# Angtian/VoGE

Measured on AMD Instinct MI355X. Metric: forward+backward frames/sec at 512^2, 50k Gaussians; ray-trace HBM GB/s vs peak, higher is better.
Workload: dtype f32; 1 GPU; cfg3_50k_512: 50000 random Gaussians (scalar sigmas), 512x512, K=40, max_point_per_bin=-1, fwd+bwd (grads to verts, sigmas, colors); launch=hip graph replay, 4 consecutive steps per graph launch, parallelism=1 gpu

## Files before the change

voge_amd/csrc/sweep_iso.h:

```cpp
#pragma once
#include <type_traits>

#include "voge_common.h"

namespace voge {

constexpr int kS2TP = 65;
constexpr int kS2TQ = 66;
constexpr int kS2Pad = 4;

struct Sweep2Stage {
  float x[64 + kS2Pad], y[64 + kS2Pad], z[64 + kS2Pad], a[64 + kS2Pad];
  union {
    float lb[64];
    int cnt[64];
  };
  int pos[64 + kS2Pad];
};
__host__ __device__ inline size_t sweep2_len_bytes(const int K) { return (sizeof(float) * (size_t)(K + 1) * kS2TP + 15) & ~(size_t)15; }
__host__ __device__ inline size_t sweep2_pos_bytes(const int K) { return (sizeof(uint16_t) * (size_t)(K + 1) * kS2TQ + 15) & ~(size_t)15; }
struct Sweep2Gen {
  float e[11][64 + kS2Pad];
};
constexpr int kS2DiagRows = 5;
__host__ __device__ inline size_t sweep2_lds_bytes(const int K, const int gen = 0) {
  return sweep2_len_bytes(K) + sweep2_pos_bytes(K) + sizeof(Sweep2Stage) +
         (gen == 1 ? sizeof(Sweep2Gen) : (gen == 2 ? sizeof(float) * kS2DiagRows * (64 + kS2Pad) : 0));
}

#ifndef VOGE_S2_EPI_B
#define VOGE_S2_EPI_B 5
#endif
#ifndef VOGE_S2_EPI_R
#define VOGE_S2_EPI_R 3
#endif
#ifndef VOGE_S2_EXIT_GROUP
#define VOGE_S2_EXIT_GROUP 16
#endif
constexpr int kExitGroup = VOGE_S2_EXIT_GROUP;

template <int GEN>
__global__ void __launch_bounds__(64)
sweep_iso_kernel(const float4 *__restrict__ cull, const float4 *__restrict__ ms, const float4 *__restrict__ evr, const float *__restrict__ rays,
                 const int *__restrict__ bin_count, const int32_t *__restrict__ bin_id, const float *__restrict__ bin_lb,
                 const int32_t *__restrict__ tl_id, const float *__restrict__ tl_lb, const int32_t *__restrict__ pool_id,
                 const float *__restrict__ pool_lb, const int *__restrict__ tl_off, const int2 *__restrict__ order,
                 const int tiles_per_img, const int nstx, const int nst, const int N, const int H, const int W, const int K,
                 const float thr_act, int32_t *__restrict__ out_idx, float *__restrict__ out_len, float *__restrict__ out_act,
                 float *__restrict__ out_dsd, int32_t *__restrict__ out_cnt,
                 const CamView cam ) {
  extern __shared__ __attribute__((aligned(16))) unsigned char smem_raw[];
  float *const Llen = reinterpret_cast<float *>(smem_raw);
  unsigned char *const Lpos_raw = smem_raw + sweep2_len_bytes(K);
  Sweep2Stage &S = *reinterpret_cast<Sweep2Stage *>(smem_raw + sweep2_len_bytes(K) + sweep2_pos_bytes(K));
  Sweep2Gen &G = *reinterpret_cast<Sweep2Gen *>(smem_raw + sweep2_len_bytes(K) + sweep2_pos_bytes(K) + sizeof(Sweep2Stage));
  auto grow = [&](const int r) -> float * { return &G.e[GEN == 2 ? (r < 2 ? r : r - 3) : r][0]; };
  auto ghas = [](const int r) { return GEN != 2 || r < 2 || (r >= 5 && r < 8); };

  const int lane = threadIdx.x;
  const int tiles_x = (W + 7) >> 3;
#ifdef VOGE_SWEEP_TIMES
  const unsigned long long ts0 = wall_clock64();
  unsigned long long ts_fill = 0, ts_cons = 0, ts1 = 0, ts2 = 0;
  unsigned st_eval = 0;
  unsigned long long ts_slow = 0; unsigned st_slow = 0, st_lanes = 0, st_moved = 0, st_far = 0;
  int dbg_moved = 0;
#endif
  const int2 slot = order[blockIdx.x];
  if (slot.x < 0) return;
  if (slot.y == 0) {
    if (out_act != nullptr) return;
    const int lin0 = slot.x & ~kPoolFlag;
    const int b = lin0 / tiles_per_img, bx = lin0 - b * tiles_per_img;
    const int ftx = bx % tiles_x, fty = bx / tiles_x;
    const int tw = min(8, W - ftx * 8), th = min(8, H - fty * 8);
    const int row_items = tw * K;
    if ((K & 3) == 0) {
      const int ipr = row_items >> 2;
      for (int it = lane; it < th * ipr; it += 64) {
        const int rr = it / ipr, j4 = it - rr * ipr;
        const size_t o = (((size_t)b * H + fty * 8 + rr) * W + (size_t)ftx * 8) * K + (size_t)j4 * 4;
        st16i<true>(out_idx + o, -1, -1, -1, -1);
        st16f<true>(out_len + o, VOGE_SENT_LEN, VOGE_SENT_LEN, VOGE_SENT_LEN, VOGE_SENT_LEN);
      }
    } else {
      for (int it = lane; it < th * row_items; it += 64) {
        const int rr = it / row_items, j = it - rr * row_items;
        const size_t o = (((size_t)b * H + fty * 8 + rr) * W + (size_t)ftx * 8) * K + j;
        out_idx[o] = -1; out_len[o] = VOGE_SENT_LEN;
      }
    }
    if (out_cnt != nullptr) {
      const int rr = lane >> 3, x = lane & 7;
      if (rr < th && x < tw) out_cnt[((size_t)b * H + fty * 8 + rr) * W + (size_t)ftx * 8 + x] = 0;
    }
    if (cam.R != nullptr && cam.rays_out != nullptr) {
      const int rr = lane >> 3, x = lane & 7;
      if (rr < th && x < tw) {
        const CamK ck = cam_load(cam, b);
        float ex, ey, ez;
        cam_ray(ck, cam_irow(cam, fty * 8 + rr), ftx * 8 + x, ex, ey, ez);
        float *o = cam.rays_out + (((size_t)b * H + fty * 8 + rr) * W + (size_t)ftx * 8 + x) * 3;
        o[0] = ex; o[1] = ey; o[2] = ez;
      }
    }
    return;
  }
  const bool pooled = (slot.x & kPoolFlag) != 0;
  const int lin = slot.x & ~kPoolFlag;
  const int b = lin / tiles_per_img, bx = lin - b * tiles_per_img;
  const int tx = bx % tiles_x, ty = bx / tiles_x;
  const int bin = (b * nst + ((ty * 8) / kST) * nstx + (tx * 8) / kST) * 4 + (((ty * 8) / kQuad) & 1) * 2 + (((tx * 8) / kQuad) & 1);
  const int tc = slot.y;
  const int bc = (tc >= 0) ? tc : ((bin_count != nullptr) ? bin_count[bin] : -1);
  const bool binned = bc >= 0;
  const int src_n = binned ? bc : N;
  const size_t list_at = pooled ? (size_t)tl_off[lin] : (size_t)lin * kTileCap;
  const int32_t *src_id = (tc >= 0) ? (pooled ? pool_id : tl_id) + list_at : (binned ? bin_id + (size_t)bin * kQCap : nullptr);
  const float *src_lb = (tc >= 0) ? (pooled ? pool_lb : tl_lb) + list_at : (binned ? bin_lb + (size_t)bin * kQCap : nullptr);
  const bool pref = tc >= 0;
  const float4 *cullb = cull + (size_t)b * N;
  const float4 *msb = ms + (size_t)b * N;
  const float4 rec_none = make_float4(0.f, 0.f, 0.f, INFINITY);
  const float4 cull_none = make_float4(0.f, 0.f, 0.f, -1.f);
  const bool h_is_id = (N <= 65536) || !binned;
  auto id_of = [&](const unsigned h) -> int { return h_is_id ? (int)h : src_id[h]; };
  const float not_full = __uint_as_float(__float_as_uint(VOGE_SENT_LEN) - 1u);
  if (lane < kS2Pad) { S.x[64 + lane] = 0.f; S.y[64 + lane] = 0.f; S.z[64 + lane] = 0.f; S.a[64 + lane] = INFINITY; }
  if (GEN && lane < kS2Pad) G.e[0][64 + lane] = __uint_as_float(0x7fc00000u);
  const float4 *evrb = GEN ? evr + (size_t)b * N * 3 : nullptr;
  bool tile_gen = false;

  Cone wcone;
  bool unit_rays = false;
  wcone.ok = false;
  const bool from_cam = cam.R != nullptr;
  CamK ck;
  if (from_cam) ck = cam_load(cam, b);
  auto ray_of = [&](const int x, const int y, float &rx, float &ry, float &rz) {
    if (from_cam) {
      cam_ray(ck, cam_irow(cam, y), x, rx, ry, rz);
    } else {
      const size_t rid = ((size_t)b * H + y) * W + x;
      rx = rays[3 * rid + 0]; ry = rays[3 * rid + 1]; rz = rays[3 * rid + 2];
    }
  };
  auto ray_setup = [&](const bool mine, const float mdx, const float mdy, const float mdz) {
    const int px = tx * 8 + (lane & 7), py = ty * 8 + (lane >> 3);
    float ox_ = mdx, oy_ = mdy, oz_ = mdz;
    if (!mine) ray_of(min(px, W - 1), min(py, H - 1), ox_, oy_, oz_);
    const RayDir u = ray_dir(ox_, oy_, oz_);
    unit_rays = __all(!u.ok || u.unit);
    wcone.ok = false;
    if (!pref) {
      const bool dirs_ok = __all(u.ok);
      const float wsx = wave_sum_dpp(u.ok ? u.ux : 0.f), wsy = wave_sum_dpp(u.ok ? u.uy : 0.f), wsz = wave_sum_dpp(u.ok ? u.uz : 0.f);
      const float n = sqrtf(fmaf(wsz, wsz, fmaf(wsy, wsy, wsx * wsx)));
      const float ax = wsx / n, ay = wsy / n, az = wsz / n;
      float smax = 0.f, cmin = 1.f;
      cone_partial(u, ax, ay, az, smax, cmin);
      wcone = cone_finish(ax, ay, az, n, wave_max(smax), wave_min(cmin), dirs_ok);
    }
  };

  auto run = [&](auto wide_tag, const int pass) {
    constexpr bool WIDE = decltype(wide_tag)::value;
    const int r = WIDE ? pass * 32 + (lane & 31) : lane;
    const int col = WIDE ? (lane & 31) : lane;
    const int px = tx * 8 + (r & 7), py = ty * 8 + (r >> 3);
    const bool valid = (px < W) && (py < H) && (!WIDE || lane < 32);
    const size_t ray_id = ((size_t)b * H + min(py, H - 1)) * W + min(px, W - 1);
    int id0 = (lane < src_n) ? (binned ? src_id[lane] : lane) : -1;
    float lb0 = (binned && lane < src_n) ? src_lb[lane] : -INFINITY;
    int id1 = (64 + lane < src_n) ? (binned ? src_id[64 + lane] : 64 + lane) : -1;
    float lb1 = (binned && 64 + lane < src_n) ? src_lb[64 + lane] : -INFINITY;
    float dx, dy, dz;
    ray_of(min(px, W - 1), min(py, H - 1), dx, dy, dz);
    if (from_cam && cam.rays_out != nullptr && valid) {
      float *o = cam.rays_out + 3 * ray_id;
      o[0] = dx; o[1] = dy; o[2] = dz;
    }
    const __amdgpu_buffer_rsrc_t rs_ms = out_rsrc(const_cast<float4 *>(msb), (unsigned)N * 16u),
                                 rs_cull = out_rsrc(const_cast<float4 *>(cullb), (unsigned)N * 16u);
    auto load_ms = [&](const int id) {
      const voge_v4f r = __builtin_amdgcn_raw_buffer_load_b128(rs_ms, id * 16, 0, 0);
      return make_float4(r[0], r[1], r[2], (id >= 0) ? r[3] : INFINITY);
    };
    auto load_cull = [&](const int id) {
      const voge_v4f r = __builtin_amdgcn_raw_buffer_load_b128(rs_cull, id * 16, 0, 0);
      return make_float4(r[0], r[1], r[2], (id >= 0) ? r[3] : -1.f);
    };
    const __amdgpu_buffer_rsrc_t rs_ev = out_rsrc(const_cast<float4 *>(GEN ? evrb : msb), GEN ? (unsigned)N * 48u : 0u);
    auto load_ev = [&](const int id, const int k) {
      const voge_v4f r = __builtin_amdgcn_raw_buffer_load_b128(rs_ev, id * 48 + 16 * k, 0, 0);
      return make_float4(r[0], r[1], r[2], r[3]);
    };
    float4 m0 = load_ms(id0);
    float4 c0 = pref ? cull_none : load_cull(id0);
    float4 ea0 = rec_none, ea1 = rec_none, ea2 = rec_none;
    if (GEN) { ea0 = load_ev(id0, 0); ea1 = load_ev(id0, 1); ea2 = load_ev(id0, 2); }
    if (pass == 0) ray_setup(!WIDE, dx, dy, dz);
    const float rdn2 = __builtin_amdgcn_rcpf((dx * dx + dy * dy) + dz * dz);
    float *const mylen = Llen + col;
    uint16_t *const mypos16 = reinterpret_cast<uint16_t *>(Lpos_raw) + col;
    uint32_t *const mypos32 = reinterpret_cast<uint32_t *>(Lpos_raw) + col;
    auto put = [&](const int row, const float len, const unsigned p) {
      mylen[__umul24((unsigned)row, (unsigned)kS2TP)] = len;
      if (WIDE) mypos32[__umul24((unsigned)row, (unsigned)(kS2TQ / 2))] = p; else mypos16[__umul24((unsigned)row, (unsigned)kS2TQ)] = (uint16_t)p;
    };
    auto len_at = [&](const int row) -> float { return mylen[__umul24((unsigned)row, (unsigned)kS2TP)]; };
    auto pos_at = [&](const int row) -> unsigned {
      return WIDE ? mypos32[__umul24((unsigned)row, (unsigned)(kS2TQ / 2))] : (unsigned)mypos16[__umul24((unsigned)row, (unsigned)kS2TQ)];
    };

    int cnt = 0;
    float worstf = valid ? not_full : __uint_as_float(0x7fc00000u);
    float tailf = -INFINITY;
    bool wdone = false;

    auto slow_insert = [&](const float len, const unsigned p) {
      const bool full = (cnt == K);
      int my_id = -1;
      auto key_le = [&](const float pl, const int row) {
        if (pl != len) return pl < len;
        if (my_id < 0) my_id = id_of(p);
        return id_of(pos_at(row)) <= my_id;
      };
      if (full && len == worstf && key_le(worstf, K - 1)) return;
      int pos = full ? K - 1 : cnt;
      float new_tail = len;
      bool first = true;
      while (pos > 0) {
        const float pl = len_at(pos - 1);
        if (key_le(pl, pos - 1)) break;
        if (first) new_tail = pl;
        put(pos, pl, pos_at(pos - 1));
        first = false;
        --pos;
      }
      put(pos, len, p);
#ifdef VOGE_SWEEP_SLOW
      dbg_moved = (full ? K - 1 : cnt) - pos;
#endif
      if (full) {
        tailf = new_tail;
        worstf = new_tail;
      } else {
        if (pos == cnt) tailf = len;
        if (++cnt == K) worstf = tailf;
      }
    };
    auto lean_insert = [&](const float len, const unsigned p, const bool slow, const int Kv) -> bool {
      const bool full = (cnt == K);
      const int top = full ? Kv - 1 : cnt;
      const int r1 = max(top - 1, 0), r2 = max(top - 2, 0), r3 = max(top - 3, 0);
      float l1 = len_at(r1), l2 = len_at(r2), l3 = len_at(r3);
      const unsigned h1 = pos_at(r1), h2 = pos_at(r2);
      l1 = (top >= 1) ? l1 : -INFINITY; l2 = (top >= 2) ? l2 : -INFINITY; l3 = (top >= 3) ? l3 : -INFINITY;
      const bool g1 = l1 > len, g2 = g1 & (l2 > len);
      const float below = g2 ? l3 : (g1 ? l2 : l1);
      const bool ok = slow & (below < len) & !(full & (len == worstf));
      const int n = (g1 ? 1 : 0) + (g2 ? 1 : 0);
      put((ok & g1) ? top : Kv, l1, h1);
      put((ok & g2) ? top - 1 : Kv, l2, h2);
      put(ok ? top - n : Kv, len, p);
      tailf = ok ? (g1 ? l1 : len) : tailf;
      cnt += (ok & !full) ? 1 : 0;
      worstf = (ok & (cnt == K)) ? tailf : worstf;
      return slow & !ok;
    };
    int Kv = K;
    asm volatile("" : "+v"(Kv));
    auto deep_insert = [&](const float len, const unsigned p, const bool slow) {
      const bool full = (cnt == K);
      bool go = slow;
      int my_id = -1;
      if (__builtin_expect(__ballot(go & full & (len == worstf)) != 0ull, 0)) {
        if (go & full & (len == worstf)) {
          my_id = id_of(p);
          if (!(my_id < id_of(pos_at(K - 1)))) go = false;
        }
      }
      int pos = full ? K - 1 : cnt;
      const int pos0 = pos;
      float top = len;
      bool walking = go, first = true;
      while (__ballot(walking) != 0ull) {
        const int r1 = max(pos - 1, 0), r2 = max(pos - 2, 0), r3 = max(pos - 3, 0), r4 = max(pos - 4, 0);
        const float l1 = len_at(r1), l2 = len_at(r2), l3 = len_at(r3), l4 = len_at(r4);
        const unsigned h1 = pos_at(r1), h2 = pos_at(r2), h3 = pos_at(r3), h4 = pos_at(r4);
        bool g1 = l1 > len, g2 = l2 > len, g3 = l3 > len, g4 = l4 > len;
        if (__builtin_expect(__ballot(walking & ((l1 == len) | (l2 == len) | (l3 == len) | (l4 == len))) != 0ull, 0)) {
          if (walking & ((l1 == len) | (l2 == len) | (l3 == len) | (l4 == len))) {
            if (my_id < 0) my_id = id_of(p);
            g1 = g1 | ((l1 == len) && id_of(h1) > my_id); g2 = g2 | ((l2 == len) && id_of(h2) > my_id);
            g3 = g3 | ((l3 == len) && id_of(h3) > my_id); g4 = g4 | ((l4 == len) && id_of(h4) > my_id);
          }
        }
        const bool c1 = walking & (pos >= 1) & g1, c2 = c1 & (pos >= 2) & g2, c3 = c2 & (pos >= 3) & g3, c4 = c3 & (pos >= 4) & g4;
        if (first) top = c1 ? l1 : len;
        first = false;
        put(c1 ? pos : Kv, l1, h1);
        put(c2 ? pos - 1 : Kv, l2, h2);
        put(c3 ? pos - 2 : Kv, l3, h3);
        put(c4 ? pos - 3 : Kv, l4, h4);
        pos -= (c1 ? 1 : 0) + (c2 ? 1 : 0) + (c3 ? 1 : 0) + (c4 ? 1 : 0);
        walking = c4;
      }
      put(go ? pos : Kv, len, p);
      if (go) {
        if (full) {
          tailf = top; worstf = top;
        } else {
          if (pos == pos0) tailf = len;
          if (++cnt == K) worstf = tailf;
        }
      }
    };

    auto commit = [&](const float len, const float act, const unsigned p) {
      const bool take = (act < thr_act) & (len <= worstf);
      const bool app = take & (len > tailf);
      put(WIDE ? (app ? cnt : Kv) : cnt, len, p);
      cnt += app ? 1 : 0;
      tailf = app ? len : tailf;
      worstf = (app & (cnt == K)) ? len : worstf;
      const bool slow = take & !app;
      if (__builtin_expect(__ballot(slow) != 0ull, 0)) {
#ifdef VOGE_SWEEP_SLOW
        const unsigned long long tss = wall_clock64();
#endif
#ifdef VOGE_SWEEP_SLOW
        dbg_moved = 0;
#endif
        if (GEN == 1) {
          deep_insert(len, p, slow);
        } else {
          const bool hard = lean_insert(len, p, slow, Kv);
          if (__builtin_expect(__ballot(hard) != 0ull, 0)) {
            if (hard) slow_insert(len, p);
          }
        }
#ifdef VOGE_SWEEP_SLOW
        ts_slow += wall_clock64() - tss; ++st_slow;
        {
          const int nl = __popcll(__ballot(slow));
          int mx = slow ? dbg_moved : 0;
          for (int o = 32; o > 0; o >>= 1) mx = max(mx, __shfl_xor(mx, o, 64));
          st_lanes += nl; st_moved += mx; st_far += (mx >= 4) ? 1 : 0;
        }
#endif
      }
    };

    auto load_id = [&](const int g) { return (g < src_n) ? (binned ? src_id[g] : g) : -1; };
    auto load_lb = [&](const int g) { return (binned && g < src_n) ? src_lb[g] : -INFINITY; };

#ifdef VOGE_SWEEP_TIMES
    ts1 = wall_clock64();
#endif
    for (int base = 0; base < src_n && !wdone; base += 64) {
      const int id = id0;
      const float lbv = lb0;
      const float4 mrec = m0, crec = c0;
      const float4 e0 = ea0, e1 = ea1, e2 = ea2;
      id0 = id1; lb0 = lb1;
      m0 = load_ms(id0);
      c0 = pref ? cull_none : load_cull(id0);
      if (GEN) { ea0 = load_ev(id0, 0); ea1 = load_ev(id0, 1); ea2 = load_ev(id0, 2); }
      id1 = load_id(base + 128 + lane);
      lb1 = load_lb(base + 128 + lane);
#ifdef VOGE_SWEEP_TIMES
      const unsigned long long tsa = wall_clock64();
#endif
      int nbuf;
      __syncthreads();
      const bool cgen = GEN && !(mrec.w == mrec.w);
      auto stage_gen = [&](const int sl) {
        const float ev[11] = {cgen ? e0.y : __uint_as_float(0x7fc00000u), e0.z, e0.w, e1.x, e1.y, e1.z, e1.w, e2.x, e2.y, e2.z, e2.w};
#pragma unroll
        for (int r = 0; r < 11; ++r)
          if (ghas(r)) grow(r)[sl] = ev[r];
      };
      const float a_st = cgen ? e0.x : mrec.w;
      if (pref) {
        S.x[lane] = mrec.x; S.y[lane] = mrec.y; S.z[lane] = mrec.z; S.a[lane] = a_st;
        S.lb[lane] = lbv;
        S.pos[lane] = h_is_id ? id : base + lane;
        if (GEN) stage_gen(lane);
        nbuf = min(64, src_n - base);
      } else {
        const bool keep = cone_keep(crec, wcone);
        const unsigned long long m = __ballot(keep);
        nbuf = __popcll(m);
        if (keep) {
          const int sl = __popcll(m & ((1ull << lane) - 1ull));
          S.x[sl] = mrec.x; S.y[sl] = mrec.y; S.z[sl] = mrec.z; S.a[sl] = a_st;
          S.lb[sl] = lbv;
          S.pos[sl] = h_is_id ? id : base + lane;
          if (GEN) stage_gen(sl);
        }
        if (lane < kS2Pad) { S.x[nbuf + lane] = 0.f; S.y[nbuf + lane] = 0.f; S.z[nbuf + lane] = 0.f; S.a[nbuf + lane] = INFINITY; }
        if (GEN && lane < kS2Pad) G.e[0][nbuf + lane] = __uint_as_float(0x7fc00000u);
      }
      __syncthreads();
      unsigned long long gmask = 0ull;
      unsigned long long dmask = 0ull;
      if (GEN) {
        const float mk = G.e[0][lane];
        gmask = __ballot(lane < nbuf && mk == mk);
        tile_gen = tile_gen || gmask != 0ull;
        if (GEN == 2) {
          dmask = gmask;
        } else if (gmask != 0ull) {
          const bool dg = G.e[2][lane] == 0.0f && G.e[3][lane] == 0.0f && G.e[4][lane] == 0.0f && G.e[8][lane] == 0.0f &&
                          G.e[9][lane] == 0.0f && G.e[10][lane] == 0.0f;
          dmask = __ballot(lane < nbuf && mk == mk && dg);
        }
      }
      const bool chunk_diag = GEN && gmask != 0ull && dmask == gmask;
#ifdef VOGE_SWEEP_TIMES
      const unsigned long long tsb = wall_clock64();
      ts_fill += tsb - tsa;
#endif
      const float lbl = S.lb[lane];
      int n = nbuf;
      float4 Xn = *reinterpret_cast<const float4 *>(&S.x[0]), Yn = *reinterpret_cast<const float4 *>(&S.y[0]),
             Zn = *reinterpret_cast<const float4 *>(&S.z[0]), An = *reinterpret_cast<const float4 *>(&S.a[0]);
      int4 Pn = *reinterpret_cast<const int4 *>(&S.pos[0]);
      float4 Evn[GEN ? 11 : 1];
      if (GEN) {
#pragma unroll
        for (int r = 0; r < 11; ++r) Evn[GEN ? r : 0] = ghas(r) ? *reinterpret_cast<const float4 *>(grow(r)) : make_float4(0.f, 0.f, 0.f, 0.f);
        if (GEN != 2 && chunk_diag) {
#pragma unroll
          for (int r = 0; r < 11; ++r)
            if (!(r < 2 || (r >= 5 && r < 8))) Evn[GEN ? r : 0] = make_float4(0.f, 0.f, 0.f, 0.f);
        }
      }
      for (int s0 = 0; s0 < n; s0 += 4) {
        if ((s0 & (kExitGroup - 1)) == 0 && binned && unit_rays && __all(!valid || cnt == K)) {
          const float wmax = wave_max(valid ? worstf : -INFINITY);
          const unsigned long long ex = __ballot(lane < nbuf && lbl > wmax);
          if (ex) {
            n = __builtin_ctzll(ex);
            wdone = true;
            if (n <= s0) break;
          }
        }
        const float4 X = Xn, Y = Yn, Z = Zn, A = An;
        const int4 P = Pn;
        const int pv[4] = {P.x, P.y, P.z, P.w};
        float len[4], act[4];
        const unsigned gbits = GEN ? (unsigned)(gmask >> s0) & 15u : 0u;
        if (GEN && gbits != 0u) {
          float4 Ev[11];
#pragma unroll
          for (int r = 0; r < 11; ++r) Ev[r] = Evn[GEN ? r : 0];
          const float qxx = dx * dx, qyy = dy * dy, qzz = dz * dz, qxy = dx * dy, qxz = dx * dz, qyz = dy * dz;
          if (gbits == 15u && ((unsigned)(dmask >> s0) & 15u) == 15u) {
#pragma unroll
            for (int h = 0; h < 2; ++h) {
              auto half = [&](const float4 v) { return h ? (v2f){v.z, v.w} : (v2f){v.x, v.y}; };
              const v2f x2 = half(X), y2 = half(Y), z2 = half(Z), s00 = half(A), s11 = half(Ev[0]), s22 = half(Ev[1]),
                        bx = half(Ev[5]), by = half(Ev[6]), bz = half(Ev[7]);
              v2f ksk = s00 * splat(qxx);
              ksk = pk_fma(s11, splat(qyy), ksk); ksk = pk_fma(s22, splat(qzz), ksk);
              v2f msk = bx * splat(dx);
              msk = pk_fma(by, splat(dy), msk); msk = pk_fma(bz, splat(dz), msk);
              const v2f t = msk * (v2f){__builtin_amdgcn_rcpf(ksk.x), __builtin_amdgcn_rcpf(ksk.y)} + splat(0.0f);
              const v2f vx = pk_fma(-t, splat(dx), x2), vy = pk_fma(-t, splat(dy), y2), vz = pk_fma(-t, splat(dz), z2);
              v2f a = s00 * (vx * vx);
              a = pk_fma(s11, vy * vy, a); a = pk_fma(s22, vz * vz, a);
              len[2 * h] = t.x; len[2 * h + 1] = t.y;
              act[2 * h] = a.x; act[2 * h + 1] = a.y;
            }
          } else if (GEN != 2 && gbits == 15u) {
#pragma unroll
            for (int h = 0; h < 2; ++h) {
              auto half = [&](const float4 v) { return h ? (v2f){v.z, v.w} : (v2f){v.x, v.y}; };
              const v2f x2 = half(X), y2 = half(Y), z2 = half(Z), s00 = half(A), s11 = half(Ev[0]), s22 = half(Ev[1]), s01 = half(Ev[2]),
                        s02 = half(Ev[3]), s12 = half(Ev[4]), bx = half(Ev[5]), by = half(Ev[6]), bz = half(Ev[7]), kx = half(Ev[8]),
                        ky = half(Ev[9]), kz = half(Ev[10]);
              v2f ksk = s00 * splat(qxx);
              ksk = pk_fma(s11, splat(qyy), ksk); ksk = pk_fma(s22, splat(qzz), ksk); ksk = pk_fma(s01, splat(qxy), ksk);
              ksk = pk_fma(s02, splat(qxz), ksk); ksk = pk_fma(s12, splat(qyz), ksk);
              v2f msk = bx * splat(dx);
              msk = pk_fma(by, splat(dy), msk); msk = pk_fma(bz, splat(dz), msk);
              const v2f t = msk * (v2f){__builtin_amdgcn_rcpf(ksk.x), __builtin_amdgcn_rcpf(ksk.y)} + splat(0.0f);
              const v2f vx = pk_fma(-t, splat(dx), x2), vy = pk_fma(-t, splat(dy), y2), vz = pk_fma(-t, splat(dz), z2);
              v2f a = s00 * (vx * vx);
              a = pk_fma(s11, vy * vy, a); a = pk_fma(s22, vz * vz, a); a = pk_fma(s01, vx * vy, a);
              a = pk_fma(s02, vx * vz, a); a = pk_fma(s12, vy * vz, a);
              v2f kd = kx * splat(dx);
              kd = pk_fma(ky, splat(dy), kd); kd = pk_fma(kz, splat(dz), kd);
              a = pk_fma(t, kd, a);
              len[2 * h] = t.x; len[2 * h + 1] = t.y;
              act[2 * h] = a.x; act[2 * h + 1] = a.y;
            }
          } else {
            const float mxs[4] = {X.x, X.y, X.z, X.w}, mys[4] = {Y.x, Y.y, Y.z, Y.w}, mzs[4] = {Z.x, Z.y, Z.z, Z.w}, avs[4] = {A.x, A.y, A.z, A.w};
#pragma unroll
            for (int q = 0; q < 4; ++q) {
              auto el = [&](const float4 v) { return q == 0 ? v.x : (q == 1 ? v.y : (q == 2 ? v.z : v.w)); };
              if ((gbits >> q) & 1u) {
                EvalRec e;
                e.s00 = avs[q]; e.s11 = el(Ev[0]); e.s22 = el(Ev[1]); e.s01 = el(Ev[2]); e.s02 = el(Ev[3]); e.s12 = el(Ev[4]);
                e.bx = el(Ev[5]); e.by = el(Ev[6]); e.bz = el(Ev[7]); e.kx = el(Ev[8]); e.ky = el(Ev[9]); e.kz = el(Ev[10]);
                const PairOut o = pair_eval_gen(mxs[q], mys[q], mzs[q], e, dx, dy, dz, qxx, qyy, qzz, qxy, qxz, qyz);
                len[q] = o.len; act[q] = o.act;
              } else {
                const float md = fmaf(mzs[q], dz, fmaf(mys[q], dy, mxs[q] * dx));
                const float t = md * rdn2;
                const float vx = fmaf(-t, dx, mxs[q]), vy = fmaf(-t, dy, mys[q]), vz = fmaf(-t, dz, mzs[q]);
                len[q] = t;
                act[q] = avs[q] * fmaf(vz, vz, fmaf(vy, vy, vx * vx));
              }
            }
          }
        } else {
#pragma unroll
        for (int h = 0; h < 2; ++h) {
          const v2f x2 = h ? (v2f){X.z, X.w} : (v2f){X.x, X.y}, y2 = h ? (v2f){Y.z, Y.w} : (v2f){Y.x, Y.y},
                    z2 = h ? (v2f){Z.z, Z.w} : (v2f){Z.x, Z.y}, a2 = h ? (v2f){A.z, A.w} : (v2f){A.x, A.y};
          const v2f md = pk_fma(z2, splat(dz), pk_fma(y2, splat(dy), x2 * splat(dx)));
          const v2f t = md * splat(rdn2);
          const v2f vx = pk_fma(-t, splat(dx), x2), vy = pk_fma(-t, splat(dy), y2), vz = pk_fma(-t, splat(dz), z2);
          const v2f a = a2 * pk_fma(vz, vz, pk_fma(vy, vy, vx * vx));
          len[2 * h] = t.x; len[2 * h + 1] = t.y;
          act[2 * h] = a.x; act[2 * h + 1] = a.y;
        }
        }
#pragma unroll
        for (int q = 0; q < 4; ++q) asm volatile("" : "+v"(len[q]), "+v"(act[q]));
        Xn = *reinterpret_cast<const float4 *>(&S.x[s0 + 4]); Yn = *reinterpret_cast<const float4 *>(&S.y[s0 + 4]);
        Zn = *reinterpret_cast<const float4 *>(&S.z[s0 + 4]); An = *reinterpret_cast<const float4 *>(&S.a[s0 + 4]);
        Pn = *reinterpret_cast<const int4 *>(&S.pos[s0 + 4]);
        if (GEN && chunk_diag) {
#pragma unroll
          for (int r = 0; r < 11; ++r)
            if (r < 2 || (r >= 5 && r < 8)) Evn[GEN ? r : 0] = *reinterpret_cast<const float4 *>(grow(r) + s0 + 4);
        } else if (GEN == 1 && gmask != 0ull) {
#pragma unroll
          for (int r = 0; r < 11; ++r) Evn[GEN ? r : 0] = *reinterpret_cast<const float4 *>(&G.e[r][s0 + 4]);
        }
#pragma unroll
        for (int q = 0; q < 4; ++q) commit(len[q], act[q], (unsigned)pv[q]);
      }
#ifdef VOGE_SWEEP_TIMES
      ts_cons += wall_clock64() - tsb;
      st_eval += min(n, nbuf);
#endif
    }
#ifdef VOGE_SWEEP_TIMES
    ts2 = wall_clock64();
#endif

    __syncthreads();
    S.cnt[lane] = valid ? cnt : 0;
    if (out_cnt != nullptr && valid) out_cnt[((size_t)b * H + py) * W + px] = cnt;
    __syncthreads();
    const int row0 = WIDE ? pass * 4 : 0;
    const int th = max(0, min(WIDE ? 4 : 8, H - ty * 8 - row0)), tw = min(8, W - tx * 8);
    const int row_items = tw * K;
    const uint16_t *const P16 = reinterpret_cast<const uint16_t *>(Lpos_raw);
    const uint32_t *const P32 = reinterpret_cast<const uint32_t *>(Lpos_raw);
    auto entry_pos = [&](const int s, const int owner) -> unsigned {
      return WIDE ? P32[s * (kS2TQ / 2) + owner] : (unsigned)P16[s * kS2TQ + owner];
    };
    const bool want_ad = out_act != nullptr;
    const int gofs = b * N;
    if ((K & 3) == 0) {
      constexpr int kEpiB = VOGE_S2_EPI_B, kEpiR = VOGE_S2_EPI_R;
      const int ipr = row_items >> 2, nitem = th * ipr;
      const float inv_ipr = 1.0f / (float)max(ipr, 1), invK = 1.0f / (float)K;
      const size_t tile_pix = ((size_t)b * H + ty * 8 + row0) * W + (size_t)tx * 8;
      int32_t *const t_idx = out_idx + tile_pix * K;
      float *const t_len = out_len + tile_pix * K;
      const unsigned h_last = (unsigned)max(src_n - 1, 0);
      const bool wt_ok = (size_t)W * (size_t)K < ((size_t)1 << 26);
      const unsigned rs_bytes = wt_ok ? (unsigned)th * (unsigned)W * (unsigned)K * 4u : 0u;
      const __amdgpu_buffer_rsrc_t rs_idx = out_rsrc(t_idx, rs_bytes), rs_len = out_rsrc(t_len, rs_bytes);
      for (int it0 = lane; it0 < nitem; it0 += 64 * kEpiB) {
        int32_t oi[kEpiB][4];
        float ol[kEpiB][4];
        unsigned rel[kEpiB];
        int nv[kEpiB];
#pragma unroll
        for (int u = 0; u < kEpiB; ++u) {
          const int it = it0 + u * 64;
          const bool in = it < nitem;
          const int itc = in ? it : 0;
          const int rr = __float2int_rz(((float)itc + 0.5f) * inv_ipr);
          const int j = (itc - rr * ipr) * 4;
          const int x = __float2int_rz(((float)j + 0.5f) * invK);
          const int sl = j - x * K;
          const int owner = rr * 8 + x;
          rel[u] = (unsigned)(rr * W + x) * (unsigned)K + (unsigned)sl;
          nv[u] = in ? max(0, min(4, S.cnt[owner] - sl)) : -1;
#pragma unroll
          for (int q = 0; q < 4; ++q) {
            const float l = Llen[(sl + q) * kS2TP + owner];
            const unsigned h = entry_pos(sl + q, owner);
            ol[u][q] = (q < nv[u]) ? l : VOGE_SENT_LEN;
            oi[u][q] = (int)h;
          }
        }
        if (h_is_id) {
#pragma unroll
          for (int u = 0; u < kEpiB; ++u)
#pragma unroll
            for (int q = 0; q < 4; ++q) oi[u][q] = (q < nv[u]) ? oi[u][q] + gofs : -1;
        } else {
          int idv[kEpiB][4];
#pragma unroll
          for (int u = 0; u < kEpiB; ++u)
#pragma unroll
            for (int q = 0; q < 4; ++q) idv[u][q] = src_id[min((unsigned)oi[u][q], h_last)];
#pragma unroll
          for (int u = 0; u < kEpiB; ++u)
#pragma unroll
            for (int q = 0; q < 4; ++q) oi[u][q] = (q < nv[u]) ? idv[u][q] + gofs : -1;
        }
        if (!want_ad) {
#pragma unroll
          for (int u = 0; u < kEpiB; ++u) {
            if (nv[u] < 0) continue;
            if (wt_ok) {
              st16i_wt(rs_idx, rel[u] * 4u, oi[u][0], oi[u][1], oi[u][2], oi[u][3]);
              st16f_wt(rs_len, rel[u] * 4u, ol[u][0], ol[u][1], ol[u][2], ol[u][3]);
            } else {
              st16i<false>(t_idx + rel[u], oi[u][0], oi[u][1], oi[u][2], oi[u][3]);
              st16f<false>(t_len + rel[u], ol[u][0], ol[u][1], ol[u][2], ol[u][3]);
            }
          }
        } else if (GEN && tile_gen) {
          float *const t_act = out_act + tile_pix * K, *const t_dsd = out_dsd + tile_pix * K;
#pragma unroll
          for (int u = 0; u < kEpiB; ++u) {
            const unsigned pr = rel[u] / (unsigned)K;
            const float *ry = rays + (tile_pix + pr) * 3;
            const float ex = ry[0], ey = ry[1], ez = ry[2];
            float4 rc[4], g0[4], g1[4], g2[4];
#pragma unroll
            for (int q = 0; q < 4; ++q) {
              const size_t gi = (size_t)((q < nv[u]) ? oi[u][q] : gofs);
              rc[q] = ms[gi]; g0[q] = evr[gi * 3]; g1[q] = evr[gi * 3 + 1]; g2[q] = evr[gi * 3 + 2];
            }
            float oa[4], od[4];
            const float dn2 = (ex * ex + ey * ey) + ez * ez;
#pragma unroll
            for (int q = 0; q < 4; ++q) {
              PairOut o;
              if (rc[q].w == rc[q].w) o = pair_eval_iso_at(rc[q].x, rc[q].y, rc[q].z, rc[q].w, ol[u][q], ex, ey, ez, dn2);
              else o = pair_eval_gen(rc[q].x, rc[q].y, rc[q].z, unpack_eval(g0[q], g1[q], g2[q]), ex, ey, ez, ex * ex, ey * ey, ez * ez,
                                     ex * ey, ex * ez, ey * ez);
              oa[q] = (q < nv[u]) ? o.act : VOGE_SENT_ACT;
              od[q] = (q < nv[u]) ? o.dsd : 0.0f;
            }
            if (nv[u] < 0) continue;
            st16i<true>(t_idx + rel[u], oi[u][0], oi[u][1], oi[u][2], oi[u][3]);
            st16f<true>(t_len + rel[u], ol[u][0], ol[u][1], ol[u][2], ol[u][3]);
            st16f<true>(t_act + rel[u], oa[0], oa[1], oa[2], oa[3]);
            st16f<true>(t_dsd + rel[u], od[0], od[1], od[2], od[3]);
          }
        } else {
          float *const t_act = out_act + tile_pix * K, *const t_dsd = out_dsd + tile_pix * K;
#pragma unroll
          for (int u0 = 0; u0 < kEpiB; u0 += kEpiR) {
            float4 rec[kEpiR][4];
            float ex[kEpiR], ey[kEpiR], ez[kEpiR];
#pragma unroll
            for (int v = 0; v < kEpiR; ++v) {
              const int u = u0 + v;
              if (u >= kEpiB) continue;
              const unsigned pr = rel[u] / (unsigned)K;
              const float *ry = rays + (tile_pix + pr) * 3;
              ex[v] = ry[0]; ey[v] = ry[1]; ez[v] = ry[2];
#pragma unroll
              for (int q = 0; q < 4; ++q) rec[v][q] = ms[(q < nv[u]) ? oi[u][q] : gofs];
            }
#pragma unroll
            for (int v = 0; v < kEpiR; ++v) {
              const int u = u0 + v;
              if (u >= kEpiB) continue;
              float oa[4], od[4];
              const float dn2 = (ex[v] * ex[v] + ey[v] * ey[v]) + ez[v] * ez[v];
#pragma unroll
              for (int q = 0; q < 4; ++q) {
                const PairOut o = pair_eval_iso_at(rec[v][q].x, rec[v][q].y, rec[v][q].z, rec[v][q].w, ol[u][q], ex[v], ey[v], ez[v], dn2);
                oa[q] = (q < nv[u]) ? o.act : VOGE_SENT_ACT;
                od[q] = (q < nv[u]) ? o.dsd : 0.0f;
              }
              if (nv[u] < 0) continue;
              st16i<true>(t_idx + rel[u], oi[u][0], oi[u][1], oi[u][2], oi[u][3]);
              st16f<true>(t_len + rel[u], ol[u][0], ol[u][1], ol[u][2], ol[u][3]);
              st16f<true>(t_act + rel[u], oa[0], oa[1], oa[2], oa[3]);
              st16f<true>(t_dsd + rel[u], od[0], od[1], od[2], od[3]);
            }
          }
        }
      }
    } else {
      constexpr int kOddU = 8;
      const float inv_ri = 1.0f / (float)max(row_items, 1), invK = 1.0f / (float)K;
      const int nit = th * row_items;
      const size_t tile_pix = ((size_t)b * H + ty * 8 + row0) * W + (size_t)tx * 8;
      int32_t *const t_idx = out_idx + tile_pix * K;
      float *const t_len = out_len + tile_pix * K;
      const unsigned h_last = (unsigned)max(src_n - 1, 0);
      for (int it0 = lane; it0 < nit; it0 += kOddU * 64) {
        int32_t oi[kOddU];
        float ol[kOddU];
        unsigned rel[kOddU], pr[kOddU];
        bool in[kOddU], on[kOddU];
#pragma unroll
        for (int u = 0; u < kOddU; ++u) {
          const int it = it0 + u * 64;
          on[u] = it < nit;
          const int itc = on[u] ? it : 0;
          const int rr = __float2int_rz(((float)itc + 0.5f) * inv_ri);
          const int j = itc - rr * row_items;
          const int x = __float2int_rz(((float)j + 0.5f) * invK);
          const int sl = j - x * K;
          const int owner = rr * 8 + x;
          pr[u] = (unsigned)(rr * W + x);
          rel[u] = pr[u] * (unsigned)K + (unsigned)sl;
          in[u] = on[u] && sl < S.cnt[owner];
          ol[u] = Llen[sl * kS2TP + owner];
          oi[u] = (int)entry_pos(sl, owner);
        }
        if (h_is_id) {
#pragma unroll
          for (int u = 0; u < kOddU; ++u) oi[u] = in[u] ? oi[u] + gofs : -1;
        } else {
          int idv[kOddU];
#pragma unroll
          for (int u = 0; u < kOddU; ++u) idv[u] = src_id[min((unsigned)oi[u], h_last)];
#pragma unroll
          for (int u = 0; u < kOddU; ++u) oi[u] = in[u] ? idv[u] + gofs : -1;
        }
#pragma unroll
        for (int u = 0; u < kOddU; ++u) ol[u] = in[u] ? ol[u] : VOGE_SENT_LEN;
        if (!want_ad) {
#pragma unroll
          for (int u = 0; u < kOddU; ++u)
            if (on[u]) { t_idx[rel[u]] = oi[u]; t_len[rel[u]] = ol[u]; }
        } else {
          float *const t_act = out_act + tile_pix * K, *const t_dsd = out_dsd + tile_pix * K;
          float oa[kOddU], od[kOddU];
#pragma unroll
          for (int u = 0; u < kOddU; ++u) {
            const float *ry = rays + (tile_pix + pr[u]) * 3;
            const float ex = ry[0], ey = ry[1], ez = ry[2];
            const size_t gi = (size_t)(in[u] ? oi[u] : gofs);
            const float4 cc = ms[gi];
            PairOut o;
            if (GEN && tile_gen && !(cc.w == cc.w)) {
              o = pair_eval_gen(cc.x, cc.y, cc.z, unpack_eval(evr[gi * 3], evr[gi * 3 + 1], evr[gi * 3 + 2]), ex, ey, ez, ex * ex, ey * ey,
                                ez * ez, ex * ey, ex * ez, ey * ez);
            } else {
              o = pair_eval_iso_at(cc.x, cc.y, cc.z, cc.w, ol[u], ex, ey, ez, (ex * ex + ey * ey) + ez * ez);
            }
            oa[u] = in[u] ? o.act : VOGE_SENT_ACT; od[u] = in[u] ? o.dsd : 0.0f;
          }
#pragma unroll
          for (int u = 0; u < kOddU; ++u)
            if (on[u]) { t_idx[rel[u]] = oi[u]; t_len[rel[u]] = ol[u]; t_act[rel[u]] = oa[u]; t_dsd[rel[u]] = od[u]; }
        }
      }
    }
  };

  if ((h_is_id ? N : src_n) <= 65536) {
    run(std::false_type{}, 0);
  } else {
    run(std::true_type{}, 0);
    run(std::true_type{}, 1);
  }
#ifdef VOGE_SWEEP_TIMES
  if (lane == 0 && b == 0 && bx < 8192) {
    unsigned long long *o = g_sweep_times + 8 * (size_t)bx;
    o[0] = ts0; o[1] = ts1; o[2] = ts_fill; o[3] = ts_cons; o[4] = ts2; o[5] = wall_clock64(); o[6] = ((unsigned long long)blockIdx.x << 32) | st_eval;
#ifdef VOGE_SWEEP_SLOW
    o[7] = (ts_slow << 32) | st_slow;
    o[2] = ((unsigned long long)st_far << 48) | ((unsigned long long)(st_moved & 0xffffu) << 32) | st_lanes;
#else
    o[7] = (unsigned long long)__builtin_amdgcn_s_getreg((4 << 0) | (0 << 6) | (31 << 11)) |
           ((unsigned long long)__builtin_amdgcn_s_getreg((20 << 0) | (0 << 6) | (31 << 11)) << 32);
#endif
  }
#endif
}

}
```

voge_amd/csrc/trace_bin.h:

```cpp
#pragma once
#include <type_traits>

#include "voge_common.h"

namespace voge {

constexpr int kST0 = 128;
constexpr int kCh = kST0 / kST;
constexpr int kBinThreads = 1024;
constexpr int kParts = 16;
constexpr int kSegCap = 512;
constexpr int kTileCap = 2048;
constexpr int kTilesPerBin = (kST / 8) * (kST / 8);
constexpr int kRankMaxBins = 4096;
static_assert(kCh * kCh == kBinThreads / 64, "one wave per super-tile of a region / per sweep tile of a super-tile");

__device__ __forceinline__ float depth_key(const float4 c, const Cone &k) {
  const float nm = __builtin_amdgcn_sqrtf(fmaf(c.z, c.z, fmaf(c.y, c.y, c.x * c.x)));
  const float R = c.w;
  if (!(R < 3e38f) || !(nm < 3e38f)) return -INFINITY;
  float kappa = -nm;
  if (k.ok && k.cs >= 0.5f && nm > 4.0f * R) {
    const float p = fmaf(c.z, k.az, fmaf(c.y, k.ay, c.x * k.ax));
    if (p > 0.0f) kappa = nm;
  }
  return kappa;
}

__device__ __forceinline__ float4 iso_cull_record(const float mx, const float my, const float mz, const float a,
                                                  const float thr_act) {
  float reach = INFINITY;
  if (a > 0.0f && a < 3e38f) {
    const float nm = __builtin_amdgcn_sqrtf(fmaf(mz, mz, fmaf(my, my, mx * mx)));
    const float r = __builtin_amdgcn_sqrtf(fmaxf(thr_act, 0.0f) * __builtin_amdgcn_rcpf(a * (1.0f - 4e-6f))) * (1.0f + 2e-5f) + 2e-5f * nm + 1e-30f;
    reach = r;
    if (!(reach >= 0.0f)) reach = INFINITY;
    if (reach < 3e38f) reach = __uint_as_float((__float_as_uint(reach) + 1u) & ~1u);
  }
  return make_float4(mx, my, mz, reach);
}

#ifdef VOGE_BIN_TIMES
__device__ unsigned long long g_bin_times[2][1024 * 8];
__device__ unsigned long long g_bin_wave[1024 * 16 * 4];
#define BIN_WTS(k) \
  if ((threadIdx.x & 63) == 0 && blockIdx.y == 0 && blockIdx.x < 1024) g_bin_wave[(blockIdx.x * 16 + (threadIdx.x >> 6)) * 4 + (k)] = wall_clock64()
#define BIN_TS(which, k) \
  if (threadIdx.x == 0 && blockIdx.y == 0 && blockIdx.x < 1024) g_bin_times[which][8 * blockIdx.x + (k)] = wall_clock64()
#else
#define BIN_TS(which, k)
#define BIN_WTS(k)
#endif

constexpr int kRoundChunks = 4;
constexpr int kRoundCap = kRoundChunks * kBinThreads;

constexpr int kExtMul = 3;
constexpr int kExtChunk = 1024;
constexpr int kExtChunks = 16;
__host__ __device__ inline int slice_cap(const int N) {
  return ((N + kParts * kBinThreads - 1) / (kParts * kBinThreads)) * kBinThreads;
}
struct BinALds {
  int arena_top;
  int extc[kCh * kCh][kExtChunks];
  int extn[kCh * kCh];
  float4 srec[kRoundCap];
  int sid[kRoundCap];
  ConeRec child[kCh * kCh];
  ConeRec region;
  ConeRec rowc[kCh];
  int use_rows;
  int cnt0[kRoundChunks][16];
  int base[kCh * kCh];
  int nS;
};

struct BinARaw {
  float4 v;
};
struct BinAView {
  float ox, oy, oz;
  float fx, fy, fz;
  bool has_f;
};
template <bool ISO_PREP>
__device__ __forceinline__ BinAView binA_view(const int b, const float *__restrict__ cam_fwd, const IsoView view,
                                              const CamView &cam = no_camera(), const CamK *ck = nullptr) {
  BinAView V;
  V.ox = V.oy = V.oz = 0.f; V.fx = V.fy = V.fz = 0.f; V.has_f = false;
  if (ISO_PREP) {
    if (view.origin != nullptr) { const float *o = view.origin + 3 * b; V.ox = o[0]; V.oy = o[1]; V.oz = o[2]; }
    if (cam_fwd != nullptr) { const float *f = cam_fwd + 3 * b; V.fx = f[0]; V.fy = f[1]; V.fz = f[2]; V.has_f = true; }
    if (cam.R != nullptr) {
      cam_origin(*ck, cam.T + 3 * b, V.ox, V.oy, V.oz);
      if (cam.behind) { const float *r = cam.R + 9 * b; V.fx = r[2]; V.fy = r[5]; V.fz = r[8]; V.has_f = true; }
    }
  }
  return V;
}
template <bool ISO_PREP>
__device__ __forceinline__ BinARaw binA_fetch(const int g, const int b, const int N, const float4 *__restrict__ cull,
                                              const float *__restrict__ mus, const float *__restrict__ isg, const IsoView view) {
  BinARaw r;
  r.v = make_float4(0.f, 0.f, 0.f, 0.f);
  if (N <= 0) return r;
  const int gc = max(g, 0);
  if (!ISO_PREP) { r.v = cull[(size_t)b * N + gc]; return r; }
  const size_t src = view.shared ? (size_t)gc : (size_t)b * N + gc;
  r.v = make_float4(mus[3 * src + 0], mus[3 * src + 1], mus[3 * src + 2], isg[src]);
  return r;
}
template <bool ISO_PREP>
__device__ __forceinline__ float4 binA_derive(const BinARaw r, const bool valid, const BinAView &V, const float thr_act,
                                              const IsoView view, float &a_out) {
  a_out = 0.f;
  if (!valid) return make_float4(0.f, 0.f, 0.f, -1.f);
  if (!ISO_PREP) return r.v;
  float mx = r.v.x, my = r.v.y, mz = r.v.z;
  if (view.origin != nullptr || view.cam_origin) { mx -= V.ox; my -= V.oy; mz -= V.oz; }
  const float a = iso_view_a(r.v.w, view.mode);
  a_out = a;
  float4 c = iso_cull_record(mx, my, mz, a, thr_act);
  if (V.has_f && fmaf(mz, V.fz, fmaf(my, V.fy, mx * V.fx)) < 0.0f) c.w = -1.0f;
  return c;
}

__host__ __device__ inline bool deal_interleaved(const int N) { return N < kParts * kBinThreads; }
__device__ __forceinline__ int slice_of(const int g, const int N) {
  return deal_interleaved(N) ? g % kParts : (g / kBinThreads) % kParts;
}

template <bool ISO_PREP>
__global__ void __launch_bounds__(kBinThreads)
binA_kernel(const ConeRec *__restrict__ cones , const int nstx, const int nsty, const int nst0x,
            const float *__restrict__ mus, const float *__restrict__ isg, const float *__restrict__ cam_fwd, const int N,
            const float thr_act, const IsoView view, float4 *__restrict__ cull, float4 *__restrict__ ms,
            int *__restrict__ seg_count , int32_t *__restrict__ seg_id ,
            float4 *__restrict__ seg_rec ,
            unsigned long long *__restrict__ pool_top ,
            int *__restrict__ seg_ext ,
            int32_t *__restrict__ ext_id , const int ext_arena,
            const CamView cam ) {
  __shared__ BinALds L;
  const int tid = threadIdx.x, lane = tid & 63, wave = tid >> 6;
  const int region = blockIdx.x / kParts, part = blockIdx.x - region * kParts;
  const int b = blockIdx.y;
  if (blockIdx.x == 0 && blockIdx.y == 0 && tid == 0) *pool_top = 0ull;
  const int rx = region % nst0x, ry = region / nst0x;
  const int nst = nstx * nsty;
  if (tid < kCh * kCh) { L.base[tid] = 0; L.extn[tid] = 0; }
  if (tid == 0) L.arena_top = 0;
  int32_t *const arena = ext_id + ((size_t)(b * (int)(gridDim.x / kParts) + region) * kParts + part) * (size_t)ext_arena;
  int ext_have = 0;
  BIN_TS(0, 0);
  const bool interleaved = deal_interleaved(N);
  const int nchunks = interleaved ? kParts * ((N + kParts * kBinThreads - 1) / (kParts * kBinThreads))
                                  : (N + kBinThreads - 1) / kBinThreads;
  const bool writes_records = ISO_PREP && region == 0;
  float4 c[kRoundChunks];
  float av[kRoundChunks];
  int gq[kRoundChunks];
  CamK ck;
  if (cam.R != nullptr) ck = cam_load(cam, b);
  const BinAView V = binA_view<ISO_PREP>(b, cam_fwd, view, cam, &ck);
  if (cam.R != nullptr && cam.origin_out != nullptr && blockIdx.x == 0 && tid == 0) {
    float ox = V.ox, oy = V.oy, oz = V.oz;
    if (!ISO_PREP) cam_origin(ck, cam.T + 3 * b, ox, oy, oz);
    cam.origin_out[3 * b] = ox; cam.origin_out[3 * b + 1] = oy; cam.origin_out[3 * b + 2] = oz;
  }
  BinARaw raw[kRoundChunks];
  auto fetch_round = [&](const int j0) {
#pragma unroll
    for (int q = 0; q < kRoundChunks; ++q) {
      const int j = j0 + q * kParts;
      const int g = interleaved ? ((j / kParts) * kBinThreads + tid) * kParts + part : j * kBinThreads + tid;
      gq[q] = (j < nchunks && g < N) ? g : -1;
      raw[q] = binA_fetch<ISO_PREP>(gq[q], b, N, cull, mus, isg, view);
    }
  };
  auto derive_round = [&]() {
#pragma unroll
    for (int q = 0; q < kRoundChunks; ++q) c[q] = binA_derive<ISO_PREP>(raw[q], gq[q] >= 0, V, thr_act, view, av[q]);
  };
  auto load_round = [&](const int j0) { fetch_round(j0); derive_round(); };
  fetch_round(part);
  if (wave == 0) {
    const int cc = lane & (kCh * kCh - 1);
    const int cx = rx * kCh + (cc & (kCh - 1)), cy = ry * kCh + cc / kCh;
    ConeRec r = {0.f, 0.f, 1.f, 1.f, 0.f, -1.f, 0.f, 0.f};
    const bool region_rect = cam.R != nullptr && cam.h <= cam.stripe_h;
    if (cam.R != nullptr) {
      const bool reg = region_rect && lane == kCh * kCh;
      const int j0 = reg ? rx * kCh * kST : cx * kST, i0 = reg ? ry * kCh * kST : cy * kST, ext = reg ? kCh * kST : kST;
      if ((cx < nstx && cy < nsty) || reg) r = cam_rect_cone(ck, cam, j0, j0 + ext - 1, i0, i0 + ext - 1);
    } else if (cx < nstx && cy < nsty) {
      r = cones[cone_super_at(b, nst, cy * nstx + cx)];
    }
    if (lane < kCh * kCh) L.child[lane] = r;
    if (region_rect) {
      if (lane == kCh * kCh) L.region = r;
      if (lane == 0) L.use_rows = 0;
    } else {
    const bool present = lane < kCh * kCh && r.ok >= 0.f;
    const float sx = wave_sum_dpp(present ? r.ax : 0.f), sy = wave_sum_dpp(present ? r.ay : 0.f), sz = wave_sum_dpp(present ? r.az : 0.f);
    const float npres = wave_sum_dpp(present ? 1.f : 0.f);
    bool ok = __all(!present || r.ok > 0.f);
    const float n = sqrtf(fmaf(sz, sz, fmaf(sy, sy, sx * sx)));
    const float ax = sx / n, ay = sy / n, az = sz / n;
    auto child_extrema = [&](const float ax_, const float ay_, const float az_, float &smax_, float &cmin_, bool &ok_) {
      smax_ = 0.f; cmin_ = 1.f;
      if (present) {
        const float ca = fmaf(r.az, az_, fmaf(r.ay, ay_, r.ax * ax_));
        const float qx = fmaf(-ca, ax_, r.ax), qy = fmaf(-ca, ay_, r.ay), qz = fmaf(-ca, az_, r.az);
        const float sa = sqrtf(fmaf(qz, qz, fmaf(qy, qy, qx * qx))) * (1.0f + 1e-6f) + 1e-7f;
        const float cl = fminf(ca, 1.0f) - 1e-7f;
        if (!(cl > 0.0f)) ok_ = false;
        cmin_ = fmaf(cl, r.cs, -sa * r.sn);
        smax_ = fmaf(fminf(ca + 1e-7f, 1.0f), r.sn, sa);
      }
    };
    float smax, cmin;
    child_extrema(ax, ay, az, smax, cmin, ok);
    ok = __all(ok);
    smax = wave_max(smax); cmin = wave_min(cmin);
    const Cone cn = cone_finish(ax, ay, az, n / fmaxf(npres, 1.f), smax, cmin, ok);
    if (lane == 0) L.region = ConeRec{cn.ax, cn.ay, cn.az, cn.cs, cn.sn, cn.ok ? 1.f : 0.f, 0.f, 0.f};
    const float widest_child = wave_max(present ? (r.ok > 0.f ? r.sn : 2.0f) : 0.f);
    if (lane == 0) L.use_rows = 0;
    if (__builtin_expect((!cn.ok || cn.sn > 8.0f * widest_child) && N < (1 << 27), 0)) {
      auto quad_sum = [](float v) { v += VOGE_DPP(v, 0xB1); v += VOGE_DPP(v, 0x4E); return v; };
      auto quad_max = [](float v) { v = fmaxf(v, VOGE_DPP(v, 0xB1)); v = fmaxf(v, VOGE_DPP(v, 0x4E)); return v; };
      auto quad_min = [](float v) { v = fminf(v, VOGE_DPP(v, 0xB1)); v = fminf(v, VOGE_DPP(v, 0x4E)); return v; };
      static_assert(kCh == 4, "a row of super-tiles is a DPP quad");
      const float qsx = quad_sum(present ? r.ax : 0.f), qsy = quad_sum(present ? r.ay : 0.f), qsz = quad_sum(present ? r.az : 0.f);
      const float qn = quad_sum(present ? 1.f : 0.f);
      const float nn = sqrtf(fmaf(qsz, qsz, fmaf(qsy, qsy, qsx * qsx)));
      const float rax = qsx / nn, ray = qsy / nn, raz = qsz / nn;
      float rs, rc;
      bool rok = !present || r.ok > 0.f;
      child_extrema(rax, ray, raz, rs, rc, rok);
      rs = quad_max(rs); rc = quad_min(rc);
      const float okf = quad_min(rok ? 1.f : 0.f);
      const Cone rcn = cone_finish(rax, ray, raz, nn / fmaxf(qn, 1.f), rs, rc, okf != 0.f);
      if (lane < kCh * kCh && (lane & 3) == 0) L.rowc[lane >> 2] = ConeRec{rcn.ax, rcn.ay, rcn.az, rcn.cs, rcn.sn, qn > 0.f ? (rcn.ok ? 1.f : 0.f) : -1.f, 0.f, 0.f};
      const float widest_row = wave_max((lane < kCh * kCh && qn > 0.f) ? (rcn.ok ? rcn.sn : 2.0f) : 0.f);
      if (lane == 0) L.use_rows = (!cn.ok || cn.sn > 1.6f * widest_row) ? 1 : 0;
    }
    }
  }
  BIN_TS(0, 6);
  derive_round();
  BIN_TS(0, 7);
  __syncthreads();
  const Cone rcone = load_cone(L.region);
  const bool use_rows = L.use_rows != 0;
  BIN_TS(0, 1);

  auto rounds = [&](auto rows_tag) {
    constexpr bool ROWS = decltype(rows_tag)::value;
    for (int j0 = part; j0 < nchunks; j0 += kParts * kRoundChunks) {
      if (j0 != part) load_round(j0);
      bool k0[kRoundChunks];
      unsigned rowm[kRoundChunks];
  #pragma unroll
      for (int q = 0; q < kRoundChunks; ++q) {
        if (writes_records && gq[q] >= 0) {
          cull[(size_t)b * N + gq[q]] = c[q];
          ms[(size_t)b * N + gq[q]] = make_float4(c[q].x, c[q].y, c[q].z, av[q]);
        }
        k0[q] = cone_keep(c[q], rcone);
        rowm[q] = 0xFu;
        if (ROWS) {
          rowm[q] = 0u;
  #pragma unroll
          for (int g = 0; g < kCh; ++g) {
            const ConeRec rr = L.rowc[g];
            if (rr.ok >= 0.f && cone_keep(c[q], load_cone(rr))) rowm[q] |= 1u << g;
          }
          k0[q] = rowm[q] != 0u;
        }
      }
      unsigned long long m0[kRoundChunks];
  #pragma unroll
      for (int q = 0; q < kRoundChunks; ++q) {
        m0[q] = __ballot(k0[q]);
        if (lane == 0) L.cnt0[q][wave] = __popcll(m0[q]);
      }
      __syncthreads();
      static_assert(kRoundChunks * 16 == 64, "one lane per (chunk, wave)");
      int nS;
      int my_off[kRoundChunks];
      {
        const int v = (&L.cnt0[0][0])[lane];
        const int x = wave_incl_scan_i32(v);
        nS = __builtin_amdgcn_readlane(x, 63);
  #pragma unroll
        for (int q = 0; q < kRoundChunks; ++q) my_off[q] = __shfl(x - v, q * 16 + wave, 64);
      }
  #pragma unroll
      for (int q = 0; q < kRoundChunks; ++q)
        if (k0[q]) {
          const int pos = my_off[q] + __popcll(m0[q] & ((1ull << lane) - 1ull));
          L.srec[pos] = c[q];
          L.sid[pos] = ROWS ? (gq[q] | (int)(rowm[q] << 27)) : gq[q];
        }
      __syncthreads();
      BIN_TS(0, 2);
      {
        const int cc = wave;
        const ConeRec cr = L.child[cc];
        if (cr.ok >= 0.f) {
          const Cone ck = load_cone(cr);
          const int ccx = rx * kCh + (cc & (kCh - 1)), ccy = ry * kCh + cc / kCh;
          const size_t seg0 = (((size_t)b * nst + ccy * nstx + ccx) * kParts + part) * kSegCap;
          int32_t *seg = seg_id + seg0;
          float4 *segr = seg_rec + seg0;
          int fill = L.base[cc];
          constexpr int kU = 4;
          for (int s0 = 0; s0 < nS; s0 += 64 * kU) {
            float4 r[kU];
            int id[kU];
  #pragma unroll
            for (int q = 0; q < kU; ++q) {
              const int si = s0 + q * 64 + lane;
              r[q] = (si < nS) ? L.srec[si] : make_float4(0.f, 0.f, 0.f, -1.f);
              id[q] = (si < nS) ? L.sid[si] : -1;
            }
            bool kp[kU];
  #pragma unroll
            for (int q = 0; q < kU; ++q) {
              bool in_row = true;
              if (ROWS) {
                in_row = id[q] >= 0 && (((unsigned)id[q] >> (27 + (cc >> 2))) & 1u) != 0u;
                id[q] = (id[q] >= 0) ? (id[q] & 0x07ffffff) : -1;
              }
              kp[q] = in_row && cone_keep(r[q], ck);
            }
            const int fill0 = fill;
  #pragma unroll
            for (int q = 0; q < kU; ++q) {
              const unsigned long long m = __ballot(kp[q]);
              if (kp[q]) {
                const int pos = fill + __popcll(m & ((1ull << lane) - 1ull));
                if (pos < kSegCap) { seg[pos] = id[q]; segr[pos] = r[q]; }
              }
              fill += __popcll(m);
            }
            if (__builtin_expect(fill > kSegCap, 0)) {
              const int need = (fill - kSegCap + kExtChunk - 1) / kExtChunk;
              while (ext_have >= 0 && ext_have < need) {
                int at = 0;
                if (lane == 0) at = atomicAdd(&L.arena_top, kExtChunk);
                at = __builtin_amdgcn_readfirstlane(at);
                if (ext_have < kExtChunks && at + kExtChunk <= ext_arena) {
                  if (lane == 0) L.extc[cc][ext_have] = at;
                  ++ext_have;
                } else {
                  ext_have = -1;
                }
              }
              wave_lds_sync();
              if (ext_have >= 0) {
                int f = fill0;
  #pragma unroll
                for (int q = 0; q < kU; ++q) {
                  const unsigned long long m = __ballot(kp[q]);
                  const int e = f + __popcll(m & ((1ull << lane) - 1ull)) - kSegCap;
                  if (kp[q] && e >= 0) arena[*lds_volatile(&L.extc[cc][e / kExtChunk]) + (e % kExtChunk)] = id[q];
                  f += __popcll(m);
                }
              }
            }
          }
          if (lane == 0) { L.base[cc] = fill; L.extn[cc] = ext_have; }
        }
      }
      BIN_TS(0, 3);
      __syncthreads();
      BIN_TS(0, 4);
    }
  };
  if (__builtin_expect(!use_rows, 1)) rounds(std::false_type{}); else rounds(std::true_type{});
  BIN_TS(0, 5);
  if (tid < kCh * kCh) {
    const int ccx = rx * kCh + (tid & (kCh - 1)), ccy = ry * kCh + tid / kCh;
    if (ccx < nstx && ccy < nsty) {
      const size_t so = ((size_t)b * nst + ccy * nstx + ccx) * kParts + part;
      const bool over = L.base[tid] > kSegCap;
      seg_count[so] = (over && L.extn[tid] < 0) ? -1 : L.base[tid];
      if (over && L.extn[tid] > 0)
        for (int q = 0; q < L.extn[tid]; ++q) seg_ext[so * kExtChunks + q] = (int)(arena - ext_id) + L.extc[tid][q];
    }
  }
}

constexpr int kQuad = 16;
constexpr int kQT = 256;
constexpr int kQCap = 3008;
constexpr int kQRec = kQCap / 2;
constexpr int kBuckets = 512;
constexpr int kTilesPerQuad = 4;
constexpr int kPoolFlag = 1 << 30;
struct BinLds {
  union {
    uint64_t keys[kQCap];
    float4 rec[kQRec];
    int hist4[kTilesPerQuad][kBuckets];
  };
  uint32_t sorted[kQCap];
  float red[4 * 8];
  union {
    int hist[kBuckets];
    int exto[kParts][kExtChunks];
  };
  uint32_t bmin[kBuckets];
  int wsum[8];
  int segn[kParts + 1];
  int extn[kParts + 1];
  unsigned ovf;
  int count;
  int nflag;
  int spill;
  float tc[kTilesPerQuad][8];
  int toff[kTilesPerQuad];
};

#ifndef VOGE_BINB_GU
#define VOGE_BINB_GU 8
#endif
constexpr int kGU = VOGE_BINB_GU;

struct BinStream {
  const float4 *cullb, *ellb, *segr;
  const int32_t *segs, *ext_id;
  const int *exto;
  int n_src, n_ext, N;
  unsigned ovf;
  Cone qcone;
};
template <bool ELL, class Sink>
__device__ __forceinline__ void bin_test_batch(const BinStream &S, const int (&gid)[kGU], const float4 (&c)[kGU], Sink &&sink) {
  bool kp[kGU], el[kGU];
  float gkey[kGU];
#pragma unroll
  for (int j = 0; j < kGU; ++j) {
    kp[j] = cone_keep(c[j], S.qcone);
    el[j] = ELL && kp[j] && cull_has_ell(c[j]);
    gkey[j] = 0.0f;
    if (ELL && __any(el[j])) {
      if (el[j]) {
        const float4 e0 = S.ellb[2 * (size_t)gid[j]], e1 = S.ellb[2 * (size_t)gid[j] + 1];
        kp[j] = cone_keep_ell(c[j], e0, e1, S.qcone);
        el[j] = kp[j];
        const float pa = fmaf(c[j].z, S.qcone.az, fmaf(c[j].y, S.qcone.ay, c[j].x * S.qcone.ax));
        gkey[j] = pa + 0.0f;
      }
    }
  }
  sink(gid, c, kp, el, gkey);
}
template <bool ELL, class Sink>
__device__ __forceinline__ void bin_stream_sources(const BinStream &S, const int *segn , const int tid, Sink &&sink) {
  int seg_p = 0, seg_lo = 0, seg_hi = segn[1];
  for (int base = 0; base < S.n_src; base += kQT * kGU) {
    int gid[kGU];
    float4 c[kGU];
#pragma unroll
    for (int j = 0; j < kGU; ++j) {
      const int i = base + j * kQT + tid;
      gid[j] = -1;
      c[j] = make_float4(0.f, 0.f, 0.f, -1.f);
      if (i < S.n_src) {
        while (i >= seg_hi) { seg_lo = seg_hi; ++seg_p; seg_hi = segn[seg_p + 1]; }
        const int o = seg_p * kSegCap + (i - seg_lo);
        gid[j] = S.segs[o];
        c[j] = S.segr[o];
      }
    }
    bin_test_batch<ELL>(S, gid, c, sink);
  }
  if (S.n_ext > 0) {
    const int *extn = segn + (kParts + 1), *exto = S.exto;
    for (int base = 0; base < S.n_ext; base += kQT * kGU) {
      int gid[kGU];
      float4 c[kGU];
#pragma unroll
      for (int j = 0; j < kGU; ++j) {
        const int i = base + j * kQT + tid;
        gid[j] = -1;
        if (i < S.n_ext) {
          int p = 0;
#pragma unroll
          for (int q = 1; q < kParts; ++q) p += (i >= extn[q]) ? 1 : 0;
          const int e = i - extn[p];
          gid[j] = S.ext_id[(size_t)exto[p * kExtChunks + e / kExtChunk] + (size_t)(e % kExtChunk)];
        }
      }
#pragma unroll
      for (int j = 0; j < kGU; ++j) c[j] = (gid[j] >= 0) ? S.cullb[gid[j]] : make_float4(0.f, 0.f, 0.f, -1.f);
      bin_test_batch<ELL>(S, gid, c, sink);
    }
  }
  if (S.ovf != 0u) {
    for (int base = 0; base < S.N; base += kQT * kGU) {
      int gid[kGU];
      float4 c[kGU];
#pragma unroll
      for (int j = 0; j < kGU; ++j) {
        const int g = base + j * kQT + tid;
        const bool ok = g < S.N && ((S.ovf >> slice_of(g, S.N)) & 1u) != 0u;
        gid[j] = ok ? g : -1;
        c[j] = ok ? S.cullb[g] : make_float4(0.f, 0.f, 0.f, -1.f);
      }
      bin_test_batch<ELL>(S, gid, c, sink);
    }
  }
}
__device__ __forceinline__ void bin_batch_slots(int *count , const int lane, const bool (&kp)[kGU], int (&slot)[kGU]) {
  unsigned long long m[kGU];
  int cw = 0;
#pragma unroll
  for (int j = 0; j < kGU; ++j) { m[j] = __ballot(kp[j]); cw += __popcll(m[j]); }
  int start = 0;
  if (cw > 0) {
    if (lane == 0) start = atomicAdd(count, cw);
    start = __builtin_amdgcn_readfirstlane(start);
  }
#pragma unroll
  for (int j = 0; j < kGU; ++j) {
    slot[j] = start + __popcll(m[j] & ((1ull << lane) - 1ull));
    start += __popcll(m[j]);
  }
}
struct BinKeys {
  float lo, scale, span, slack;
  bool flagged;
};
__device__ __forceinline__ int bin_bucket_of(const BinKeys &Kk, const float v) {
  return (v > -INFINITY) ? 1 + min(kBuckets - 2, max(0, (int)((v - Kk.lo) * Kk.scale))) : 0;
}
__device__ __forceinline__ float bin_own_bound(const BinStream &S, const size_t g) {
  const float4 cj = S.cullb[g], e0 = S.ellb[2 * g], e1 = S.ellb[2 * g + 1];
  float bnd = -INFINITY;
  if (S.qcone.ok) {
    const float pa = fmaf(cj.z, S.qcone.az, fmaf(cj.y, S.qcone.ay, cj.x * S.qcone.ax));
    const float nm1 = fabsf(cj.x) + fabsf(cj.y) + fabsf(cj.z);
    const float t = pa - ell_support(e0, e1, S.qcone.ax, S.qcone.ay, S.qcone.az) - 4e-6f * nm1;
    bnd = (t >= 0.0f) ? t : t / S.qcone.cs;
    bnd = bnd - 1e-5f * fabsf(bnd) - 1e-30f;
  }
  return bnd;
}
__device__ __forceinline__ void bin_bmin_suffix(uint32_t *bmin, int *wsum, const int tid) {
  const int lane = tid & 63, wave = tid >> 6;
  uint32_t m4[2];
#pragma unroll
  for (int q = 0; q < 2; ++q) m4[q] = bmin[2 * tid + q];
  m4[0] = min(m4[0], m4[1]);
  uint32_t x = m4[0];
#pragma unroll
  for (int o = 1; o < 64; o <<= 1) {
    const uint32_t y = __shfl_down(x, o, 64);
    if (lane + o < 64) x = min(x, y);
  }
  if (lane == 0) wsum[4 + wave] = (int)x;
  __syncthreads();
  uint32_t later = 0xffffffffu;
  {
    const uint32_t nxt = __shfl_down(x, 1, 64);
    later = (lane < 63) ? nxt : 0xffffffffu;
    for (int w = wave + 1; w < 4; ++w) later = min(later, (uint32_t)wsum[4 + w]);
  }
#pragma unroll
  for (int q = 0; q < 2; ++q) bmin[2 * tid + q] = min(m4[q], later);
}
__device__ __forceinline__ float bin_len_bound(const BinKeys &Kk, const uint32_t *bmin, const float v) {
  float edge = -INFINITY;
  int qb = 0;
  if (v > -INFINITY) {
    const int q = min(kBuckets - 2, max(0, (int)((v - Kk.lo) * Kk.scale)));
    edge = fminf(v, Kk.lo + (float)q * (Kk.span / (float)(kBuckets - 2)) - 4e-6f * Kk.span);
    qb = 1 + q;
  }
  const float lb_sphere = (edge > -INFINITY) ? edge - Kk.slack - 1e-5f * fabsf(edge) - 1e-30f : -INFINITY;
  return Kk.flagged ? fminf(lb_sphere, ord2f(bmin[qb])) : lb_sphere;
}

struct BinLong {
  BinStream S;
  BinKeys Kk;
  Cone tcone;
  bool tile_ok;
  int tile, quad, total;
  unsigned long long *pool_top;
  int *tl_off, *tl_count, *q_count;
  const int *seg_ext;
  int bin;
  int pool_cap;
  int32_t *pool_id;
  float *pool_lb;
  int2 *my_order;
};
template <bool ELL>
__device__ __forceinline__ void binB_long_path(const BinLong A, BinLds &L) {
  const int tid = threadIdx.x, lane = tid & 63, wave = tid >> 6;
  const BinStream &S = A.S;
  const int total = A.total;
  __syncthreads();
  for (int i = tid; i < kTilesPerQuad * kBuckets; i += kQT) (&L.hist4[0][0])[i] = 0;
  if (S.n_ext > 0) {
    const int p = tid / kExtChunks, q = tid % kExtChunks;
    const int ne = L.extn[p + 1] - L.extn[p];
    L.exto[p][q] = (q * kExtChunk < ne) ? A.seg_ext[((size_t)A.bin * kParts + p) * kExtChunks + q] : 0;
  }
  if (lane == 0) {
    L.tc[wave][0] = A.tcone.ax; L.tc[wave][1] = A.tcone.ay; L.tc[wave][2] = A.tcone.az; L.tc[wave][3] = A.tcone.cs;
    L.tc[wave][4] = A.tcone.sn; L.tc[wave][5] = (A.tcone.ok || !A.tile_ok) ? 1.0f : 0.0f;
    L.tc[wave][6] = A.tile_ok ? 1.0f : 0.0f;
  }
  if (tid == 0) {
    const unsigned long long at64 = atomicAdd(A.pool_top, (unsigned long long)total);
    int at = (at64 + (unsigned long long)total <= (unsigned long long)A.pool_cap) ? (int)at64 : -1;
    L.toff[0] = at;
    L.count = 0;
  }
  __syncthreads();
  const int surv_at = L.toff[0];
  bool pooled = surv_at >= 0;
  int tile_n[kTilesPerQuad] = {0, 0, 0, 0};
  if (pooled) {
    int32_t *sv_id = A.pool_id + surv_at;
    float *sv_key = A.pool_lb + surv_at;
    bin_stream_sources<ELL>(S, L.segn, tid, [&](const int (&g)[kGU], const float4 (&cj)[kGU], const bool (&kp)[kGU],
                                            const bool (&el)[kGU], const float (&gkey)[kGU]) {
      int slot[kGU];
      bin_batch_slots(&L.count, lane, kp, slot);
#pragma unroll
      for (int j = 0; j < kGU; ++j) {
        if (kp[j]) {
          sv_id[slot[j]] = (int32_t)((uint32_t)g[j] | (el[j] ? 0x80000000u : 0u));
          sv_key[slot[j]] = el[j] ? gkey[j] : depth_key(cj[j], S.qcone);
        }
      }
    });
    __threadfence_block();
    __syncthreads();
    BIN_TS(1, 2);
    auto tile_mask = [&](const size_t g, const float4 cj, const bool el) {
      unsigned mk = 0u;
#pragma unroll 1
      for (int t = 0; t < kTilesPerQuad; ++t) {
        Cone tk;
        tk.ax = L.tc[t][0]; tk.ay = L.tc[t][1]; tk.az = L.tc[t][2]; tk.cs = L.tc[t][3]; tk.sn = L.tc[t][4];
        tk.ok = L.tc[t][5] != 0.0f;
        bool k2 = (L.tc[t][6] != 0.0f) && cone_keep(cj, tk);
        if (k2 && el) k2 = cone_keep_ell(cj, S.ellb[2 * g], S.ellb[2 * g + 1], tk);
        mk |= k2 ? (1u << t) : 0u;
      }
      return mk;
    };
    for (int i = tid; i < total; i += kQT) {
      const uint32_t word = (uint32_t)sv_id[i];
      const size_t g = word & 0x7fffffffu;
      const bool el = ELL && (word & 0x80000000u) != 0u;
      const int q = bin_bucket_of(A.Kk, sv_key[i]);
      const unsigned mk = tile_mask(g, S.cullb[g], el);
#pragma unroll
      for (int t = 0; t < kTilesPerQuad; ++t)
        if ((mk >> t) & 1u) atomicAdd(&L.hist4[t][q], 1);
      if (el) atomicMin(&L.bmin[q], f2ord(bin_own_bound(S, g)));
    }
    __syncthreads();
    for (int t = 0; t < kTilesPerQuad; ++t) {
      const int2 v = *reinterpret_cast<const int2 *>(&L.hist4[t][2 * tid]);
      const int s4 = v.x + v.y;
      int x = s4;
#pragma unroll
      for (int o = 1; o < 64; o <<= 1) {
        const int y = __shfl_up(x, o, 64);
        if (lane >= o) x += y;
      }
      if (lane == 63) L.wsum[wave] = x;
      __syncthreads();
      int off = x - s4;
      for (int w = 0; w < wave; ++w) off += L.wsum[w];
      tile_n[t] = L.wsum[0] + L.wsum[1] + L.wsum[2] + L.wsum[3];
      *reinterpret_cast<int2 *>(&L.hist4[t][2 * tid]) = make_int2(off, off + v.x);
      __syncthreads();
    }
    if (ELL && A.Kk.flagged) bin_bmin_suffix(L.bmin, L.wsum, tid);
    if (tid == 0) {
      const int need = tile_n[0] + tile_n[1] + tile_n[2] + tile_n[3];
      const unsigned long long at64 = (need > 0) ? atomicAdd(A.pool_top, (unsigned long long)need) : 0ull;
      int at = (at64 + (unsigned long long)need <= (unsigned long long)A.pool_cap) ? (int)at64 : -1;
#pragma unroll
      for (int t = 0; t < kTilesPerQuad; ++t) { L.toff[t] = at; if (at >= 0) at += tile_n[t]; }
    }
    __syncthreads();
    pooled = L.toff[0] >= 0;
    BIN_TS(1, 3);
    if (pooled) {
      for (int i = tid; i < total; i += kQT) {
        const uint32_t word = (uint32_t)sv_id[i];
        const size_t g = word & 0x7fffffffu;
        const bool el = ELL && (word & 0x80000000u) != 0u;
        const float kv = sv_key[i];
        const int q = bin_bucket_of(A.Kk, kv);
        const unsigned mk = tile_mask(g, S.cullb[g], el);
        if (mk == 0u) continue;
        const float lbv = bin_len_bound(A.Kk, L.bmin, kv);
#pragma unroll
        for (int t = 0; t < kTilesPerQuad; ++t) {
          if ((mk >> t) & 1u) {
            const size_t pos = (size_t)L.toff[t] + (size_t)atomicAdd(&L.hist4[t][q], 1);
            A.pool_id[pos] = (int32_t)g;
            A.pool_lb[pos] = lbv;
          }
        }
      }
    }
  }
  if (lane == 0 && A.tile_ok) {
    A.tl_count[A.tile] = pooled ? tile_n[wave] : -1;
    A.tl_off[A.tile] = pooled ? L.toff[wave] : -1;
  }
  __syncthreads();
  if (lane == 0) L.wsum[wave] = A.tile_ok ? (pooled ? tile_n[wave] : 0x7fffffff) : -1;
  __syncthreads();
  if (lane == 0) {
    const int mine = L.wsum[wave];
    int slot = 0;
    for (int w = 0; w < kTilesPerQuad; ++w) {
      const int o = L.wsum[w];
      slot += (o > mine || (o == mine && w < wave)) ? 1 : 0;
    }
    A.my_order[slot] = make_int2(A.tile_ok ? (pooled ? (A.tile | kPoolFlag) : A.tile) : -1, pooled ? mine : -1);
  }
  if (tid == 0) A.q_count[A.quad] = pooled ? -2 : -1;
  BIN_TS(1, 4);
}


#ifndef VOGE_BINB_WPE
#define VOGE_BINB_WPE 4
#endif
template <bool ELL>
__global__ void __launch_bounds__(kQT) __attribute__((amdgpu_waves_per_eu(VOGE_BINB_WPE, VOGE_BINB_WPE)))
binB_kernel(const float4 *__restrict__ cull, const float4 *__restrict__ ell, const int *__restrict__ seg_count,
            const int32_t *__restrict__ seg_id, const float4 *__restrict__ seg_rec,
            const ConeRec *__restrict__ cones ,
            const int N, const int H, const int W,
            const int nstx, const int nsty, const int nbin_total,
            int *__restrict__ q_count, int32_t *__restrict__ q_id, float *__restrict__ q_lb,
            int *__restrict__ tl_count, int32_t *__restrict__ tl_id, float *__restrict__ tl_lb,
            int2 *__restrict__ order ,
            unsigned long long *__restrict__ pool_top, const int pool_cap, int32_t *__restrict__ pool_id, float *__restrict__ pool_lb,
            int *__restrict__ tl_off, const int *__restrict__ seg_ext, const int32_t *__restrict__ ext_id,
            const int K, int32_t *__restrict__ out_idx, float *__restrict__ out_len, float *__restrict__ out_act,
            float *__restrict__ out_dsd, int32_t *__restrict__ out_cnt, float *__restrict__ out_weight,
            int64_t *__restrict__ out_valid, const CamView cam ) {
  __shared__ BinLds L;
  const int tid = threadIdx.x, lane = tid & 63, wave = tid >> 6;
  BIN_TS(1, 7);
  const int b = blockIdx.y;
  const int binl = blockIdx.x >> 2, qq = blockIdx.x & 3;
  const int stx = binl % nstx, sty = binl / nstx;
  const int bin = b * nstx * nsty + binl;
  const int quad = bin * 4 + qq;
  const int tiles_x = (W + 7) >> 3, tiles_y = (H + 7) >> 3;
  const int tx = stx * (kST / 8) + (qq & 1) * 2 + (wave & 1), ty = sty * (kST / 8) + (qq >> 1) * 2 + (wave >> 1);
  const bool tile_ok = tx < tiles_x && ty < tiles_y;
  const int tile = b * tiles_x * tiles_y + ty * tiles_x + tx;

  ConeRec tcr, qcr;
  if (cam.R != nullptr) {
    const CamK ck = cam_load(cam, b);
    cam_two_cones(ck, cam, tx * 8, ty * 8, 8, stx * kST + (qq & 1) * kQuad, sty * kST + (qq >> 1) * kQuad, kQuad, tcr, qcr);
  } else {
    tcr = cones[cone_tile_at(b, (size_t)nstx * nsty, binl, ((qq >> 1) * 2 + (wave >> 1)) * 4 + (qq & 1) * 2 + (wave & 1))];
    qcr = cones[cone_quad_at(b, (size_t)nstx * nsty, binl, qq)];
  }
  const int my_cnt = (tid < kParts) ? seg_count[(size_t)bin * kParts + tid] : 0;
  const bool ranked = nbin_total <= kRankMaxBins;
  const int4 est0 = (ranked && tid < nbin_total) ? *reinterpret_cast<const int4 *>(seg_count + (size_t)tid * kParts) : make_int4(0, 0, 0, 0);
  const int4 est_mine = ranked ? *reinterpret_cast<const int4 *>(seg_count + (size_t)bin * kParts) : make_int4(0, 0, 0, 0);
  const Cone tcone = load_cone(tcr), qcone = load_cone(qcr);
  {
    if (tid == 0) { L.count = 0; L.nflag = 0; L.spill = 0; }
    if (wave == 0) {
      int c = (lane < kParts) ? my_cnt : 0;
      const unsigned long long ofm = __ballot(lane < kParts && c < 0);
      if (c < 0) c = 0;
      int e = 0;
      if (c > kSegCap) { e = c - kSegCap; c = kSegCap; }
      int xc = c, xe = e;
#pragma unroll
      for (int o = 1; o < kParts; o <<= 1) {
        const int yc = __shfl_up(xc, o, 64), ye = __shfl_up(xe, o, 64);
        if (lane >= o) { xc += yc; xe += ye; }
      }
      if (lane < kParts) { L.segn[lane] = xc - c; L.extn[lane] = xe - e; }
      if (lane == kParts - 1) { L.segn[kParts] = xc; L.extn[kParts] = xe; }
      if (lane == 0) L.ovf = (unsigned)ofm;
    }
    __syncthreads();
    auto load_ext_tables = [&]() {
      static_assert(kParts * kExtChunks == kQT, "one thread per (slice, chunk)");
      const int p = tid / kExtChunks, q = tid % kExtChunks;
      const int ne = L.extn[p + 1] - L.extn[p];
      L.exto[p][q] = (q * kExtChunk < ne) ? seg_ext[((size_t)bin * kParts + p) * kExtChunks + q] : 0;
    };
    if (L.extn[kParts] > 0) load_ext_tables();
  }
  BIN_TS(1, 0);

  BIN_TS(1, 6);
  int rank = bin;
  {
    auto est_of = [](const int4 v) {
      return (v.x < 0 ? kSegCap : v.x) + (v.y < 0 ? kSegCap : v.y) + (v.z < 0 ? kSegCap : v.z) + (v.w < 0 ? kSegCap : v.w);
    };
    auto estimate = [&](const int q) { return est_of(*reinterpret_cast<const int4 *>(seg_count + (size_t)q * kParts)); };
    if (ranked) {
      const int mine = est_of(est_mine);
      int ahead = 0;
      for (int q = tid; q < nbin_total; q += kQT) {
        const int e = (q == tid) ? est_of(est0) : estimate(q);
        ahead += (e > mine || (e == mine && q < bin)) ? 1 : 0;
      }
      ahead = (int)wave_sum_dpp((float)ahead);
      if (lane == 0) L.wsum[wave] = ahead;
      __syncthreads();
      rank = L.wsum[0] + L.wsum[1] + L.wsum[2] + L.wsum[3];
      __syncthreads();
    }
  }
  int2 *my_order = order + (size_t)rank * kTilesPerBin + qq * kTilesPerQuad;
  const int n_src = L.segn[kParts];
  const unsigned ovf = L.ovf;
  const float4 *cullb = cull + (size_t)b * N;
  const float4 *ellb = ell + (size_t)b * N * 2;
  const int32_t *segs = seg_id + (size_t)bin * kParts * kSegCap;
  const float4 *segr = seg_rec + (size_t)bin * kParts * kSegCap;
  float rmax = 0.0f;
  float klo = INFINITY, khi = -INFINITY;
  bool any_el = false;
  BinStream S;
  S.cullb = cullb; S.ellb = ellb; S.segr = segr; S.segs = segs; S.n_src = n_src; S.N = N; S.ovf = ovf; S.qcone = qcone;
  S.ext_id = ext_id; S.n_ext = L.extn[kParts]; S.exto = &L.exto[0][0];
  bin_stream_sources<ELL>(S, L.segn, tid, [&](const int (&g)[kGU], const float4 (&cj)[kGU], const bool (&kp)[kGU],
                                          const bool (&el)[kGU], const float (&gkey)[kGU]) {
    int slot[kGU];
    bin_batch_slots(&L.count, lane, kp, slot);
#pragma unroll
    for (int j = 0; j < kGU; ++j) {
      if (kp[j]) {
        if (!el[j] && cj[j].w < 3e38f) rmax = fmaxf(rmax, cj[j].w);
        const float kv = el[j] ? gkey[j] : depth_key(cj[j], qcone);
        if (kv > -INFINITY) { klo = fminf(klo, kv); khi = fmaxf(khi, kv); }
        if (slot[j] < kQCap) L.keys[slot[j]] = ((uint64_t)f2ord(kv) << 32) | (uint32_t)g[j] | (el[j] ? 0x80000000u : 0u);
        any_el = any_el || el[j];
      }
    }
  });
  BIN_TS(1, 1);
  if (__any(any_el) && lane == 0) L.nflag = 1;
  float hi = wave_max(khi), lo = wave_min(klo), rm = wave_max(rmax);
  if (lane == 0) { L.red[wave * 8 + 0] = hi; L.red[wave * 8 + 1] = lo; L.red[wave * 8 + 2] = rm; }
  if (S.n_ext > 0) __syncthreads();
  for (int i = tid; i < kBuckets; i += kQT) { L.hist[i] = 0; L.bmin[i] = f2ord(INFINITY); }
  __syncthreads();
  const int total = L.count;
  hi = fmaxf(fmaxf(L.red[0], L.red[8]), fmaxf(L.red[16], L.red[24]));
  lo = fminf(fminf(L.red[1], L.red[9]), fminf(L.red[17], L.red[25]));
  rm = fmaxf(fmaxf(L.red[2], L.red[10]), fmaxf(L.red[18], L.red[26]));
  const float span = fmaxf(hi - lo, 1e-20f);
  const float scale = (float)(kBuckets - 2) / span;
  const bool flagged = ELL && L.nflag != 0;
  BinKeys Kk;
  Kk.lo = lo; Kk.scale = scale; Kk.span = span; Kk.slack = 1.13f * rm * (1.0f + 1e-5f); Kk.flagged = flagged;
  auto bucket_of = [&](const uint64_t k) { return bin_bucket_of(Kk, ord2f((uint32_t)(k >> 32))); };
  if (__builtin_expect(total > kQCap, 0)) {
    BinLong A;
    A.S = S; A.Kk = Kk; A.tcone = tcone; A.tile_ok = tile_ok; A.tile = tile; A.quad = quad; A.total = total;
    A.pool_top = pool_top; A.tl_off = tl_off; A.tl_count = tl_count; A.q_count = q_count; A.pool_cap = pool_cap;
    A.pool_id = pool_id; A.pool_lb = pool_lb; A.my_order = my_order; A.seg_ext = seg_ext; A.bin = bin;
    binB_long_path<ELL>(A, L);
  } else {
  for (int i = tid; i < total; i += kQT) {
    const uint64_t kk = L.keys[i];
    const int q = bucket_of(kk);
    atomicAdd(&L.hist[q], 1);
    if (ELL && ((uint32_t)kk & 0x80000000u)) atomicMin(&L.bmin[q], f2ord(bin_own_bound(S, (size_t)((uint32_t)kk & 0x7fffffffu))));
  }
  __syncthreads();
  {
    static_assert(kBuckets == 2 * kQT, "two buckets per thread");
    const int2 v = *reinterpret_cast<const int2 *>(&L.hist[2 * tid]);
    const int s4 = v.x + v.y;
    int x = s4;
#pragma unroll
    for (int o = 1; o < 64; o <<= 1) {
      const int y = __shfl_up(x, o, 64);
      if (lane >= o) x += y;
    }
    if (lane == 63) L.wsum[wave] = x;
    __syncthreads();
    int off = x - s4;
    for (int w = 0; w < wave; ++w) off += L.wsum[w];
    *reinterpret_cast<int2 *>(&L.hist[2 * tid]) = make_int2(off, off + v.x);
  }
  __syncthreads();
  BIN_TS(1, 2);
  for (int i = tid; i < total; i += kQT) {
    const uint64_t kk = L.keys[i];
    L.sorted[atomicAdd(&L.hist[bucket_of(kk)], 1)] = (uint32_t)kk;
  }
  if (flagged) {
    __syncthreads();
    bin_bmin_suffix(L.bmin, L.wsum, tid);
  }
  __syncthreads();
  for (int i0 = 0; i0 < min(total, kQRec); i0 += kQT * kGU) {
    float4 c[kGU];
#pragma unroll
    for (int j = 0; j < kGU; ++j) {
      const int i = i0 + j * kQT + tid;
      c[j] = (i < min(total, kQRec)) ? cullb[L.sorted[i] & 0x7fffffffu] : make_float4(0.f, 0.f, 0.f, -1.f);
    }
#pragma unroll
    for (int j = 0; j < kGU; ++j) {
      const int i = i0 + j * kQT + tid;
      if (i < min(total, kQRec)) L.rec[i] = c[j];
    }
  }
  __syncthreads();
  BIN_TS(1, 3);
  auto len_bound = [&](const uint32_t word, const float4 cr) {
    const float v = (ELL && (word & 0x80000000u)) ? fmaf(cr.z, qcone.az, fmaf(cr.y, qcone.ay, cr.x * qcone.ax)) + 0.0f
                                         : depth_key(cr, qcone);
    return bin_len_bound(Kk, L.bmin, v);
  };

  int kept = 0;
  if (tile_ok) {
    int32_t *oid = tl_id + (size_t)tile * kTileCap;
    float *olb = tl_lb + (size_t)tile * kTileCap;
    BIN_WTS(0);
#ifndef VOGE_BINB_FU
#define VOGE_BINB_FU 4
#endif
    constexpr int kFU = VOGE_BINB_FU;
    for (int base = 0; base < total; base += 64 * kFU) {
      uint32_t k[kFU];
      float4 cr[kFU];
#pragma unroll
      for (int q = 0; q < kFU; ++q) {
        const int i = base + q * 64 + lane;
        k[q] = (i < total) ? L.sorted[i] : 0u;
        cr[q] = make_float4(0.f, 0.f, 0.f, -1.f);
        if (i < total) cr[q] = L.rec[min(i, kQRec - 1)];
        if (__any(i >= kQRec && i < total)) {
          if (i >= kQRec && i < total) cr[q] = cullb[k[q] & 0x7fffffffu];
        }
      }
      bool kp[kFU];
#pragma unroll
      for (int q = 0; q < kFU; ++q) kp[q] = cone_keep(cr[q], tcone);
#pragma unroll
      for (int q = 0; q < kFU; ++q) {
        if (base + q * 64 >= total) break;
        const uint32_t word = k[q];
        const bool el = ELL && kp[q] && (word & 0x80000000u);
        if (__any(el)) {
          if (el) {
            const size_t g = word & 0x7fffffffu;
            kp[q] = cone_keep_ell(cr[q], ellb[2 * g], ellb[2 * g + 1], tcone);
          }
        }
        const unsigned long long m = __ballot(kp[q]);
        if (kp[q]) {
          const int pos = kept + __popcll(m & ((1ull << lane) - 1ull));
          if (pos < kTileCap) { oid[pos] = (int32_t)(word & 0x7fffffffu); olb[pos] = len_bound(word, cr[q]); }
        }
        kept += __popcll(m);
      }
    }
    BIN_WTS(1);
    if (lane == 0) {
      if (kept > kTileCap) { tl_count[tile] = -1; L.spill = 1; }
      else tl_count[tile] = kept;
    }
  }
  if (lane == 0) L.wsum[wave] = tile_ok ? min(kept, kTileCap + 1) : -1;
  __syncthreads();
  BIN_TS(1, 4);
  if (lane == 0) {
    const int mine = L.wsum[wave];
    int slot = 0;
    for (int w = 0; w < kTilesPerQuad; ++w) {
      const int o = L.wsum[w];
      slot += (o > mine || (o == mine && w < wave)) ? 1 : 0;
    }
    my_order[slot] = make_int2(tile_ok ? tile : -1, (mine > kTileCap) ? -1 : mine);
  }
  if (L.spill) {
    int32_t *oid = q_id + (size_t)quad * kQCap;
    float *olb = q_lb + (size_t)quad * kQCap;
    for (int i = tid; i < total; i += kQT) {
      const uint32_t word = L.sorted[i];
      oid[i] = (int32_t)(word & 0x7fffffffu);
      float4 crec = L.rec[min(i, kQRec - 1)];
      if (i >= kQRec) crec = cullb[word & 0x7fffffffu];
      olb[i] = len_bound(word, crec);
    }
  }
  if (tid == 0) q_count[quad] = L.spill ? total : -2;
  }
  for (int w = 0; w < kTilesPerQuad && out_idx != nullptr; ++w) {
    if (L.wsum[w] != 0) continue;
    const int ftx = stx * (kST / 8) + (qq & 1) * 2 + (w & 1), fty = sty * (kST / 8) + (qq >> 1) * 2 + (w >> 1);
    const int tw = min(8, W - ftx * 8), th = min(8, H - fty * 8);
    const int row_items = tw * K;
    if ((K & 3) == 0) {
      const int ipr = row_items >> 2;
      for (int it = tid; it < th * ipr; it += kQT) {
        const int rr = it / ipr, j4 = it - rr * ipr;
        const size_t o = (((size_t)b * H + fty * 8 + rr) * W + (size_t)ftx * 8) * K + (size_t)j4 * 4;
        st16i<true>(out_idx + o, -1, -1, -1, -1);
        st16f<true>(out_len + o, VOGE_SENT_LEN, VOGE_SENT_LEN, VOGE_SENT_LEN, VOGE_SENT_LEN);
        if (out_weight != nullptr) {
          *reinterpret_cast<float4 *>(out_weight + o) = make_float4(0.f, 0.f, 0.f, 0.f);
        } else if (out_act != nullptr) {
          st16f<true>(out_act + o, VOGE_SENT_ACT, VOGE_SENT_ACT, VOGE_SENT_ACT, VOGE_SENT_ACT);
          st16f<true>(out_dsd + o, 0.f, 0.f, 0.f, 0.f);
        }
      }
    } else {
      for (int it = tid; it < th * row_items; it += kQT) {
        const int rr = it / row_items, j = it - rr * row_items;
        const size_t o = (((size_t)b * H + fty * 8 + rr) * W + (size_t)ftx * 8) * K + j;
        out_idx[o] = -1; out_len[o] = VOGE_SENT_LEN;
        if (out_act != nullptr) { out_act[o] = VOGE_SENT_ACT; out_dsd[o] = 0.0f; }
        if (out_weight != nullptr) out_weight[o] = 0.0f;
      }
    }
    if (tid < th * 8) {
      const int rr = tid >> 3, x = tid & 7;
      const size_t pix = ((size_t)b * H + fty * 8 + rr) * W + (size_t)ftx * 8 + x;
      if (x < tw && out_cnt != nullptr) out_cnt[pix] = 0;
      if (x < tw && out_valid != nullptr) out_valid[pix] = 0;
    }
  }
  BIN_TS(1, 5);
}

}
```

voge_amd/csrc/trace_fwd.hip:

```cpp
#include "voge_common.h"

namespace voge {

__device__ inline double lambda_min_sym3(double a00, double a11, double a22, double a01,
                                         double a02, double a12) {
  const double p1 = a01 * a01 + a02 * a02 + a12 * a12;
  if (p1 == 0.0) return fmin(a00, fmin(a11, a22));
  const double q = (a00 + a11 + a22) / 3.0;
  const double b00 = a00 - q, b11 = a11 - q, b22 = a22 - q;
  const double p2 = b00 * b00 + b11 * b11 + b22 * b22 + 2.0 * p1;
  const double p = sqrt(p2 / 6.0);
  const double ip = 1.0 / p;
  const double c00 = b00 * ip, c11 = b11 * ip, c22 = b22 * ip;
  const double c01 = a01 * ip, c02 = a02 * ip, c12 = a12 * ip;
  double r = 0.5 * (c00 * (c11 * c22 - c12 * c12) - c01 * (c01 * c22 - c12 * c02) +
                    c02 * (c01 * c12 - c11 * c02));
  r = fmin(1.0, fmax(-1.0, r));
  const double phi = acos(r) / 3.0;
  return q + 2.0 * p * cos(phi + 2.0943951023931953);
}

__device__ __forceinline__ void prep_one(const int g, const float *__restrict__ mus, const float *__restrict__ isg,
                                         const float *__restrict__ cam_fwd, const int N, const float thr_act,
                                         const int iso_in, float4 *__restrict__ cull, float4 *__restrict__ evr,
// ... 930 lines not shown
  const size_t pix = ((size_t)b * H + py) * W + px;
  const float dx = rays[3 * pix + 0], dy = rays[3 * pix + 1], dz = rays[3 * pix + 2];
  const float qxx = dx * dx, qyy = dy * dy, qzz = dz * dz, qxy = dx * dy, qxz = dx * dz, qyz = dy * dz;
  const int by = min(py / bin_size, BH - 1), bx = min(px / bin_size, BW - 1);
  const int32_t *lst = bins + (((size_t)b * BH + by) * BW + bx) * M;
  uint64_t *mykeys = keys + lane;
  int cnt = 0;
  uint64_t worst = ~0ull, tail = 0ull;
  for (int m = 0; m < M; ++m) {
    const int p = lst[m];
    if (p < 0 || p >= P) continue;
    float A[9];
#pragma unroll
    for (int i = 0; i < 9; ++i) A[i] = isg[9 * (size_t)p + i];
    const float mx = mus[3 * (size_t)p], my = mus[3 * (size_t)p + 1], mz = mus[3 * (size_t)p + 2];
    const EvalRec e = make_eval(mx, my, mz, A);
    const PairOut o = pair_eval(mx, my, mz, e, dx, dy, dz, qxx, qyy, qzz, qxy, qxz, qyz);
    if (o.act < thr_act && o.len < VOGE_SENT_LEN) {
      const uint64_t key = ((uint64_t)f2ord(o.len) << 32) | (uint32_t)p;
      if (key < worst) topk_insert(mykeys, 64, K, cnt, worst, tail, key);
    }
  }
  for (int s = 0; s < K; ++s) {
    int32_t oi = -1;
    float ol = VOGE_SENT_LEN, oa = VOGE_SENT_ACT, od = 0.0f;
    if (s < cnt) {
      const uint64_t key = mykeys[(size_t)s * 64];
      oi = (int32_t)(uint32_t)key;
      float A[9];
#pragma unroll
      for (int i = 0; i < 9; ++i) A[i] = isg[9 * (size_t)oi + i];
      const float mx = mus[3 * (size_t)oi], my = mus[3 * (size_t)oi + 1], mz = mus[3 * (size_t)oi + 2];
      const EvalRec e = make_eval(mx, my, mz, A);
      const PairOut o = pair_eval(mx, my, mz, e, dx, dy, dz, qxx, qyy, qzz, qxy, qxz, qyz);
      ol = ord2f((uint32_t)(key >> 32));
      oa = o.act;
      od = o.dsd;
    }
    out_idx[pix * K + s] = oi;
    out_len[pix * K + s] = ol;
    out_act[pix * K + s] = oa;
    out_dsd[pix * K + s] = od;
  }
  if (out_cnt != nullptr) out_cnt[pix] = cnt;
}

struct TraceWs {
  float4 *cull, *evr, *ms, *ell;
  ConeRec *cones;
  int *seg_count;
  int32_t *seg_id;
  int *q_count;
  int32_t *q_id;
  float *q_lb;
  int *tl_count;
  int32_t *tl_id;
  float *tl_lb;
  float4 *seg_rec;
  int2 *order;
  unsigned long long *pool_top;
  int32_t *pool_id;
  float *pool_lb;
  int *tl_off;
  int pool_cap;
  int *seg_ext;
  int32_t *ext_id;
  int ext_arena;
  int nstx, nsty, nst0x, nst0y, nbin;
};

static size_t trace_pool_entries(const size_t P) {
  const size_t want = 32 * P;
  return want < ((size_t)1 << 20) ? ((size_t)1 << 20) : (want > ((size_t)1 << 30) ? ((size_t)1 << 30) : want);
}

static size_t align256(size_t v) { return (v + 255) & ~(size_t)255; }
constexpr int kPoolSlots = 64;
constexpr size_t kPoolTail = 512;
static unsigned long long *trace_pool_slots(void *workspace, const size_t workspace_bytes) {
  return reinterpret_cast<unsigned long long *>(reinterpret_cast<char *>(workspace) + ((workspace_bytes - kPoolTail) & ~(size_t)255));
}

static size_t trace_ws_layout(int B, int N, int H, int W, void *base, TraceWs *ws) {
  const size_t P = (size_t)B * N;
  const int nstx = (W + kST - 1) / kST, nsty = (H + kST - 1) / kST;
  const size_t nbin = (size_t)B * nstx * nsty;
  const size_t ntile = (size_t)B * ((W + 7) / 8) * ((H + 7) / 8);
  size_t off = 0;
  char *p = reinterpret_cast<char *>(base);
  auto take = [&](size_t bytes) { char *q = p ? p + off : nullptr; off += align256(bytes); return q; };
  char *c = take(P * 16), *e = take(P * 48), *m4 = take(P * 16), *el = take(P * 32), *cn = take(cone_records(1, nbin) * sizeof(ConeRec)),
       *sc = take(nbin * kParts * 4), *si = take(nbin * kParts * (size_t)kSegCap * 4), *bc = take(nbin * 4 * 4),
       *bi = take(nbin * 4 * kQCap * 4), *bl = take(nbin * 4 * kQCap * 4), *tc = take(ntile * 4),
       *ti = take(ntile * kTileCap * 4), *tl = take(ntile * kTileCap * 4), *sr = take(nbin * kParts * (size_t)kSegCap * 16),
       *cq = take(nbin * kTilesPerBin * 8 * 2);
  const size_t npool = trace_pool_entries(P);
  char *pi = take(npool * 4), *pl = take(npool * 4), *to = take(ntile * 4);
  const int nst0x = (W + kST0 - 1) / kST0, nst0y = (H + kST0 - 1) / kST0;
  size_t arena = (size_t)kExtMul * slice_cap(N);
  if ((size_t)B * nst0x * nst0y * kParts * arena > (size_t)0x7fffffff) arena = 0;
  char *se = take(nbin * kParts * kExtChunks * 4), *ei = take((size_t)B * nst0x * nst0y * kParts * arena * 4);
  if (ws) {
    ws->seg_ext = reinterpret_cast<int *>(se); ws->ext_id = reinterpret_cast<int32_t *>(ei); ws->ext_arena = (int)arena;
    ws->pool_top = nullptr ; ws->pool_id = reinterpret_cast<int32_t *>(pi);
    ws->pool_lb = reinterpret_cast<float *>(pl); ws->tl_off = reinterpret_cast<int *>(to);
    ws->pool_cap = (int)npool;
    ws->cull = reinterpret_cast<float4 *>(c); ws->evr = reinterpret_cast<float4 *>(e);
    ws->ms = reinterpret_cast<float4 *>(m4); ws->ell = reinterpret_cast<float4 *>(el);
    ws->cones = reinterpret_cast<ConeRec *>(cn);
    ws->seg_count = reinterpret_cast<int *>(sc); ws->seg_id = reinterpret_cast<int32_t *>(si);
    ws->q_count = reinterpret_cast<int *>(bc); ws->q_id = reinterpret_cast<int32_t *>(bi);
    ws->q_lb = reinterpret_cast<float *>(bl);
    ws->tl_count = reinterpret_cast<int *>(tc); ws->tl_id = reinterpret_cast<int32_t *>(ti);
    ws->tl_lb = reinterpret_cast<float *>(tl);
    ws->seg_rec = reinterpret_cast<float4 *>(sr); ws->order = reinterpret_cast<int2 *>(cq);
    ws->nstx = nstx; ws->nsty = nsty;
    ws->nst0x = (W + kST0 - 1) / kST0; ws->nst0y = (H + kST0 - 1) / kST0;
    ws->nbin = (int)nbin;
  }
  return off;
}

#ifdef VOGE_AB
static std::atomic<int> g_sweep_variant{0};
#endif
template <bool ISO>
static int launch_trace(const TraceWs &ws, const ConeRec *cones, const float *rays, int B, int N, int H, int W, int K,
                        float thr_act, int32_t *idx, float *len, float *act, float *dsd, int32_t *cnt, float occ,
                        hipStream_t st, const CamView &cam, const bool diag = false) {
  constexpr int T = 64;
  const int gen = ISO ? 0 : (diag ? 2 : 1);
  const auto sweep = ISO ? sweep_iso_kernel<0> : (diag ? sweep_iso_kernel<2> : sweep_iso_kernel<1>);
#ifdef VOGE_AB
  const bool v2 = g_sweep_variant.load(std::memory_order_relaxed) != 1;
#else
  constexpr bool v2 = true;
#endif
  const size_t lds2 = sweep2_lds_bytes(K, gen);
  {
    static DynLdsCache cache2[2];
    if (v2) {
      const int rc = ensure_dynamic_lds(reinterpret_cast<const void *>(sweep), lds2, cache2[diag ? 1 : 0]);
      if (rc) return rc;
    }
  }
#ifdef VOGE_AB
  const size_t lds = ((sizeof(uint64_t) * (size_t)(K + 1) * (T + 1) + 15) & ~(size_t)15) + ((sizeof(TraceLds<T, ISO>) + 15) & ~(size_t)15);
  if (!v2) {
    static DynLdsCache cache;
    const int rc = ensure_dynamic_lds(reinterpret_cast<const void *>(trace_fwd_kernel<1, ISO>), lds, cache);
    if (rc) return rc;
  }
#endif
  hipLaunchKernelGGL(binB_kernel<!ISO>, dim3(ws.nstx * ws.nsty * 4, B), dim3(kQT), 0, st, ws.cull, ws.ell, ws.seg_count, ws.seg_id, ws.seg_rec,
                     cones, N, H, W, ws.nstx, ws.nsty, ws.nbin, ws.q_count, ws.q_id, ws.q_lb, ws.tl_count, ws.tl_id, ws.tl_lb,
                     ws.order, ws.pool_top, ws.pool_cap, ws.pool_id, ws.pool_lb, ws.tl_off, ws.seg_ext, ws.ext_id, K,
                     (v2 && act == nullptr) ? nullptr : idx , len, act, dsd, cnt,
                     nullptr, nullptr, cam);
  {
    int rc = launch_status();
    if (rc) return rc;
  }
  const int2 *order = ws.order;
  dim3 grid(ws.nbin * kTilesPerBin);
  if (v2) {
    hipLaunchKernelGGL(sweep, grid, dim3(T), lds2, st, ws.cull, ws.ms, ws.evr, rays, ws.q_count, ws.q_id, ws.q_lb, ws.tl_id,
                       ws.tl_lb, ws.pool_id, ws.pool_lb, ws.tl_off, order, ((W + 7) / 8) * ((H + 7) / 8), ws.nstx, ws.nstx * ws.nsty, N, H, W, K,
                       thr_act, idx, len, act, dsd, cnt, cam);
    return launch_status();
  }
#ifdef VOGE_AB
  if (cam.R != nullptr) return VOGE_ERR_BAD_ARG;
  hipLaunchKernelGGL((trace_fwd_kernel<1, ISO>), grid, dim3(T), lds, st, ws.cull, ws.evr, ws.ms, rays, ws.q_count, ws.q_id, ws.q_lb,
                     ws.tl_count, ws.tl_id, ws.tl_lb, ws.pool_id, ws.pool_lb, ws.tl_off, order, ((W + 7) / 8) * ((H + 7) / 8), ws.nstx,
                     ws.nstx * ws.nsty, N, H, W, K, thr_act, idx, len, act, dsd, cnt, occ, nullptr, nullptr);
#endif
  return launch_status();
}

}

using namespace voge;

#ifdef VOGE_SWEEP_TIMES
extern "C" int voge_debug_sweep_stats(unsigned long long *out16) {
  hipError_t e = hipMemcpyFromSymbol(out16, HIP_SYMBOL(voge::g_sweep_stats), sizeof(unsigned long long) * 16);
  if (e != hipSuccess) return (int)e;
  unsigned long long z[16] = {0};
  return (int)hipMemcpyToSymbol(HIP_SYMBOL(voge::g_sweep_stats), z, sizeof(z));
}
#endif
#ifdef VOGE_SWEEP_TIMES
extern "C" int voge_debug_sweep_times(unsigned long long *out, int n_wg) {
  return (int)hipMemcpyFromSymbol(out, HIP_SYMBOL(voge::g_sweep_times), sizeof(unsigned long long) * 8 * (size_t)n_wg);
}
#endif

#ifdef VOGE_BIN_TIMES
extern "C" int voge_debug_bin_wave(unsigned long long *out, int n_wg) {
  return (int)hipMemcpyFromSymbol(out, HIP_SYMBOL(voge::g_bin_wave), sizeof(unsigned long long) * 64 * (size_t)n_wg);
}
extern "C" int voge_debug_bin_times(unsigned long long *out, int which, int n_wg) {
  return (int)hipMemcpyFromSymbol(out, HIP_SYMBOL(voge::g_bin_times), sizeof(unsigned long long) * 8 * (size_t)n_wg,
                                  sizeof(unsigned long long) * 8 * 1024 * (size_t)which);
}
#endif

#ifdef VOGE_AB
extern "C" int voge_debug_sweep_variant(int variant) {
  if (variant < 0 || variant > 1) return VOGE_ERR_BAD_ARG;
  voge::g_sweep_variant.store(variant, std::memory_order_relaxed);
  return 0;
}
#endif

constexpr size_t kTraceWsCap = (size_t)1 << 30;
static size_t trace_ws_bytes(const int nb, const int N, const int H, const int W) {
  return trace_ws_layout(nb, N, H, W, nullptr, nullptr) + 256 + kPoolTail;
}
static int trace_views_that_fit(const int B, const int N, const int H, const int W, const size_t bytes) {
  int nb = 1;
  for (int step = B; step >= 1; step >>= 1)
    while (nb + step <= B && trace_ws_bytes(nb + step, N, H, W) <= bytes) nb += step;
  return nb;
}
extern "C" size_t voge_trace_workspace_bytes(int B, int N, int H, int W) {
  if (B <= 0 || N < 0 || H <= 0 || W <= 0) return 0;
  return trace_ws_bytes(trace_views_that_fit(B, N, H, W, kTraceWsCap), N, H, W);
}

extern "C" int voge_trace_pool_usage(const void *workspace, size_t workspace_bytes, int B, int N, int H, int W, int *used,
                                     int *capacity) {
  if (!workspace || !used || !capacity || B <= 0 || N < 0 || H <= 0 || W <= 0) return VOGE_ERR_BAD_ARG;
  if (workspace_bytes < trace_ws_bytes(1, N, H, W)) return VOGE_ERR_WORKSPACE;
  const int per = trace_views_that_fit(B, N, H, W, workspace_bytes);
  const int nchunks = (B + per - 1) / per;
  unsigned long long tops[kPoolSlots];
  const hipError_t e = hipMemcpy(tops, trace_pool_slots(const_cast<void *>(workspace), workspace_bytes), sizeof(tops), hipMemcpyDeviceToHost);
  if (e != hipSuccess) return (int)e;
  unsigned long long top = 0ull;
  for (int c = 0; c < nchunks && c < kPoolSlots; ++c) top = tops[c] > top ? tops[c] : top;
  TraceWs ws;
  trace_ws_layout(per, N, H, W, const_cast<void *>(workspace), &ws);
  *capacity = ws.pool_cap;
  if (nchunks > 1 && B % per != 0) {
    trace_ws_layout(B % per, N, H, W, const_cast<void *>(workspace), &ws);
    *capacity = ws.pool_cap < *capacity ? ws.pool_cap : *capacity;
  }
  *used = top > 0x7fffffffull ? 0x7fffffff : (int)top;
  return 0;
}

extern "C" int voge_ray_cones(const float *rays, int B, int H, int W, float *cones, voge_stream_t stream);
extern "C" int voge_composite_fwd_iso(const int32_t *idx, const int32_t *cnt, const float *len, const float *records,
                                      const float *rays, float occ, long npix, int K, float *weight, int64_t *valid_num,
                                      voge_stream_t stream);

__global__ void __launch_bounds__(256) idx_rebase_kernel(int32_t *__restrict__ idx, const size_t n4, const int off) {
  for (size_t i = (size_t)blockIdx.x * blockDim.x + threadIdx.x; i < n4; i += (size_t)gridDim.x * blockDim.x) {
    int4 v = reinterpret_cast<int4 *>(idx)[i];
    v.x = v.x >= 0 ? v.x + off : v.x; v.y = v.y >= 0 ? v.y + off : v.y; v.z = v.z >= 0 ? v.z + off : v.z; v.w = v.w >= 0 ? v.w + off : v.w;
    reinterpret_cast<int4 *>(idx)[i] = v;
  }
}
__global__ void __launch_bounds__(256) idx_rebase1_kernel(int32_t *__restrict__ idx, const size_t n, const int off) {
  for (size_t i = (size_t)blockIdx.x * blockDim.x + threadIdx.x; i < n; i += (size_t)gridDim.x * blockDim.x) {
    const int v = idx[i];
    if (v >= 0) idx[i] = v + off;
  }
}

static int trace_chunk_fwd(const int iso_in, const IsoView view, const float *mus, const float *isigmas, const float *rays,
                           const float *cam_fwd, const float *cones_in, int B, int N, int H, int W, int K,
                           float thr_act, void *workspace, int32_t *idx, float *len, float *act, float *dsd, int32_t *cnt,
                           voge_stream_t stream, float occ, float *weight, int64_t *valid_num, float *records, const CamView &cam,
                           unsigned long long *pool_top);

static int trace_topk_fwd_impl(const int iso_in, const IsoView view, const float *mus, const float *isigmas, const float *rays,
                               const float *cam_fwd, const float *cones_in, int B, int N, int H, int W, int K,
                               float thr_act, void *workspace, size_t workspace_bytes,
                               int32_t *idx, float *len, float *act, float *dsd, int32_t *cnt,
                               voge_stream_t stream, float occ = 1.0f, float *weight = nullptr, int64_t *valid_num = nullptr,
                               float *records = nullptr, const CamView cam = no_camera()) {
  if (B < 0 || N < 0 || H < 0 || W < 0 || K <= 0) return VOGE_ERR_BAD_ARG;
  if (K > VOGE_MAX_K) return VOGE_ERR_K_TOO_LARGE;
  if ((size_t)B * H * W == 0) return 0;
  if (cam.R != nullptr) {
    if (rays || cones_in || cam_fwd || act || dsd || !cam.T || !cam.focal || !cam.pp || cam.stripe_h <= 0 || cam.pitch < 0 ||
        cam.h != H || cam.W != W || (weight != nullptr && !cam.rays_out))
      return VOGE_ERR_BAD_ARG;
  } else if (!rays) {
    return VOGE_ERR_BAD_ARG;
  }
  if (!idx || !len || !workspace || (act == nullptr) != (dsd == nullptr)) return VOGE_ERR_BAD_ARG;
  if (act == nullptr && !((iso_in ? (weight != nullptr || records != nullptr) : (weight == nullptr && records != nullptr)) &&
                          cnt != nullptr && (long)B * N < (1l << 26)))
    return VOGE_ERR_BAD_ARG;
  if (N > 0 && (!mus || !isigmas)) return VOGE_ERR_BAD_ARG;
  if (workspace_bytes < trace_ws_bytes(1, N, H, W)) return VOGE_ERR_WORKSPACE;
  if (sizeof(uint64_t) * (size_t)(K + 1) * 65 + 16 + sizeof(TraceLds<64, false>) > 160 * 1024) return VOGE_ERR_K_TOO_LARGE;
  const int per = trace_views_that_fit(B, N, H, W, workspace_bytes);
  const size_t npv = (size_t)H * W;
  const size_t nst = (size_t)((W + kST - 1) / kST) * ((H + kST - 1) / kST);
  const size_t stride_mu = view.shared ? 0 : (size_t)N * 3;
  const size_t stride_sg = iso_in ? (view.shared ? 0 : (size_t)N)
                                  : (view.gen_kind ? (view.sigma_shared ? 0 : (size_t)N * (view.gen_kind == 2 ? 9 : 3)) : (size_t)N * 9);
  for (int b0 = 0; b0 < B; b0 += per) {
    const int nb = (B - b0 < per) ? B - b0 : per;
    IsoView v = view;
    if (v.origin != nullptr) v.origin += 3 * (size_t)b0;
    if (v.quats != nullptr && !v.sigma_shared) v.quats += 4 * (size_t)b0 * N;
    auto at = [&](auto *p, const size_t per_view) { return p ? p + (size_t)b0 * per_view : p; };
    if (cam.R != nullptr) v.cam_origin = 1;
    CamView cv = cam;
    cv.R = at(cam.R, 9); cv.T = at(cam.T, 3); cv.focal = at(cam.focal, 2); cv.pp = at(cam.pp, 2);
    cv.origin_out = at(cam.origin_out, 3); cv.rays_out = at(cam.rays_out, npv * 3);
    const int rc = trace_chunk_fwd(iso_in, v, at(mus, stride_mu), at(isigmas, stride_sg), at(rays, npv * 3), at(cam_fwd, 3),
                                   at(cones_in, nst * kConeRecsPerST * (sizeof(ConeRec) / sizeof(float))), nb, N, H, W, K, thr_act, workspace,
                                   at(idx, npv * K), at(len, npv * K), at(act, npv * K), at(dsd, npv * K), at(cnt, npv), stream, occ,
                                   at(weight, npv * K), at(valid_num, npv), at(records, (size_t)N * (iso_in ? 4 : (view.gen_kind == 1 ? 8 : 12))), cv,
                                   trace_pool_slots(workspace, workspace_bytes) + ((b0 / per) < kPoolSlots ? (b0 / per) : kPoolSlots - 1));
// ... 240 lines not shown
```

voge_amd/csrc/voge_common.h:

```cpp
#pragma once
#include <hip/hip_runtime.h>
#include <stdint.h>

#include <atomic>

#include "voge_hip.h"

#define VOGE_WAVE 64

#define VOGE_SENT_LEN 1e10f
#define VOGE_SENT_ACT 1e10f

namespace voge {

struct EvalRec {
  float s00, s11, s22, s01, s02, s12;
  float bx, by, bz;
  float kx, ky, kz;
};
static_assert(sizeof(EvalRec) == 48, "EvalRec must be 3 x float4");

__device__ __forceinline__ float fast_div(const float a, const float b) { return a * __builtin_amdgcn_rcpf(b); }

constexpr uint32_t kIsoFlag = 0x7fc0a150u;
// ... 256 lines not shown
    keys[(unsigned)pos * (unsigned)stride] = key;
    if (full) {
      tail = top;
      worst = top;
    } else if (++cnt == K) {
      worst = tail;
    }
  }
}

__device__ __forceinline__ float wave_sum(float v) {
#pragma unroll
  for (int o = 32; o > 0; o >>= 1) v += __shfl_xor(v, o, 64);
  return v;
}
typedef float voge_v4f __attribute__((ext_vector_type(4)));
typedef int voge_v4i __attribute__((ext_vector_type(4)));
template <bool NT>
__device__ __forceinline__ void st16f(float *p, const float a, const float b, const float c, const float d) {
  const voge_v4f v = {a, b, c, d};
  if (NT) __builtin_nontemporal_store(v, reinterpret_cast<voge_v4f *>(p)); else *reinterpret_cast<voge_v4f *>(p) = v;
}
__device__ __forceinline__ __amdgpu_buffer_rsrc_t out_rsrc(void *base, const unsigned bytes) {
  return __builtin_amdgcn_make_buffer_rsrc(base, 0, (int)bytes, 0x00020000);
}
__device__ __forceinline__ void st16f_wt(const __amdgpu_buffer_rsrc_t r, const unsigned byte_off, const float a, const float b,
                                         const float c, const float d) {
  const voge_v4f v = {a, b, c, d};
  __builtin_amdgcn_raw_buffer_store_b128(v, r, (int)byte_off, 0, 16 );
}
__device__ __forceinline__ void st16i_wt(const __amdgpu_buffer_rsrc_t r, const unsigned byte_off, const int a, const int b,
                                         const int c, const int d) {
  const voge_v4i v = {a, b, c, d};
  __builtin_amdgcn_raw_buffer_store_b128(v, r, (int)byte_off, 0, 16 );
}
template <bool NT>
__device__ __forceinline__ void st16i(int32_t *p, const int a, const int b, const int c, const int d) {
  const voge_v4i v = {a, b, c, d};
  if (NT) __builtin_nontemporal_store(v, reinterpret_cast<voge_v4i *>(p)); else *reinterpret_cast<voge_v4i *>(p) = v;
}
#define VOGE_DPP(v, ctrl) __int_as_float(__builtin_amdgcn_update_dpp(0, __float_as_int(v), ctrl, 0xF, 0xF, true))
#define VOGE_LANE(v, l) __int_as_float(__builtin_amdgcn_readlane(__float_as_int(v), l))
__device__ __forceinline__ float wave_max(float v) {
  v = fmaxf(v, VOGE_DPP(v, 0xB1));
  v = fmaxf(v, VOGE_DPP(v, 0x4E));
  v = fmaxf(v, VOGE_DPP(v, 0x141));
  v = fmaxf(v, VOGE_DPP(v, 0x140));
  return fmaxf(fmaxf(VOGE_LANE(v, 0), VOGE_LANE(v, 16)), fmaxf(VOGE_LANE(v, 32), VOGE_LANE(v, 48)));
}
__device__ __forceinline__ float wave_min(float v) {
  v = fminf(v, VOGE_DPP(v, 0xB1));
  v = fminf(v, VOGE_DPP(v, 0x4E));
  v = fminf(v, VOGE_DPP(v, 0x141));
  v = fminf(v, VOGE_DPP(v, 0x140));
  return fminf(fminf(VOGE_LANE(v, 0), VOGE_LANE(v, 16)), fminf(VOGE_LANE(v, 32), VOGE_LANE(v, 48)));
}
__device__ __forceinline__ int wave_incl_scan_i32(int v) {
  v += __builtin_amdgcn_update_dpp(0, v, 0x111, 0xF, 0xF, true);
  v += __builtin_amdgcn_update_dpp(0, v, 0x112, 0xF, 0xF, true);
  v += __builtin_amdgcn_update_dpp(0, v, 0x114, 0xF, 0xF, true);
  v += __builtin_amdgcn_update_dpp(0, v, 0x118, 0xF, 0xF, true);
  v += __builtin_amdgcn_update_dpp(0, v, 0x142, 0xA, 0xF, false);
  v += __builtin_amdgcn_update_dpp(0, v, 0x143, 0xC, 0xF, false);
  return v;
}
__device__ __forceinline__ float wave_sum_dpp(float v) {
  v += VOGE_DPP(v, 0xB1);
  v += VOGE_DPP(v, 0x4E);
  v += VOGE_DPP(v, 0x141);
  v += VOGE_DPP(v, 0x140);
  return (VOGE_LANE(v, 0) + VOGE_LANE(v, 16)) + (VOGE_LANE(v, 32) + VOGE_LANE(v, 48));
}

struct Cone {
  float ax, ay, az, cs, sn;
  bool ok;
};

__device__ __forceinline__ bool cone_keep(const float4 c, const Cone &k) {
  if (c.w < 0.0f) return false;
  const float p = fmaf(c.z, k.az, fmaf(c.y, k.ay, c.x * k.ax));
  const float rx = fmaf(-p, k.ax, c.x), ry = fmaf(-p, k.ay, c.y), rz = fmaf(-p, k.az, c.z);
  const float q = __builtin_amdgcn_sqrtf(fmaf(rz, rz, fmaf(ry, ry, rx * rx)));
  const float gap = fmaf(q, k.cs, -fabsf(p) * k.sn);
  return !k.ok || !(gap > c.w);
}

constexpr int kST = 32;

struct RayDir {
  float ux, uy, uz;
  bool ok;
  bool unit;
};
__device__ __forceinline__ RayDir ray_dir(const float dx, const float dy, const float dz) {
  RayDir r;
  const float dn2 = fmaf(dz, dz, fmaf(dy, dy, dx * dx));
  const float inv = 1.0f / sqrtf(dn2);
  r.ok = (dn2 > 0.0f) && (inv < 3e38f) && (inv == inv);
  r.unit = fabsf(dn2 - 1.0f) < 1e-4f;
  r.ux = dx * inv; r.uy = dy * inv; r.uz = dz * inv;
  return r;
}
__device__ __forceinline__ void cone_partial(const RayDir &u, const float ax, const float ay, const float az,
                                             float &smax, float &cmin) {
  const float cl = fmaf(u.uz, az, fmaf(u.uy, ay, u.ux * ax));
  const float rx = fmaf(-cl, ax, u.ux), ry = fmaf(-cl, ay, u.uy), rz = fmaf(-cl, az, u.uz);
  const float sl = sqrtf(fmaf(rz, rz, fmaf(ry, ry, rx * rx)));
  smax = fmaxf(smax, u.ok ? sl : 2.0f);
  cmin = fminf(cmin, u.ok ? cl : -1.0f);
}
__device__ __forceinline__ Cone cone_finish(const float ax, const float ay, const float az, const float n,
                                            const float smax, const float cmin, const bool all_ok) {
  Cone c;
  c.ax = ax; c.ay = ay; c.az = az;
  c.sn = smax * (1.0f + 1e-5f) + 1e-7f;
  c.cs = cmin - 1e-6f;
  c.ok = all_ok && (n > 1e-3f) && (cmin > 0.05f) && (c.sn == c.sn);
  return c;
}

struct ConeRec {
  float ax, ay, az, cs, sn, ok, pad0, pad1;
};
__device__ __forceinline__ Cone load_cone(const ConeRec &r) {
  Cone c;
  c.ax = r.ax; c.ay = r.ay; c.az = r.az; c.cs = r.cs; c.sn = r.sn; c.ok = r.ok > 0.f;
  return c;
}

struct Mat3 {
  float m[9];
};
__device__ __forceinline__ Mat3 inv3(const float *R) {
  Mat3 o;
  const float a = R[0], b = R[1], c = R[2], d = R[3], e = R[4], f = R[5], g = R[6], h = R[7], i = R[8];
  const float A = e * i - f * h, B = -(d * i - f * g), C = d * h - e * g;
  const float det = a * A + b * B + c * C;
  const float id = 1.0f / det;
  o.m[0] = A * id;               o.m[1] = -(b * i - c * h) * id;  o.m[2] = (b * f - c * e) * id;
  o.m[3] = B * id;               o.m[4] = (a * i - c * g) * id;   o.m[5] = -(a * f - c * d) * id;
  o.m[6] = C * id;               o.m[7] = -(a * h - b * g) * id;  o.m[8] = (a * e - b * d) * id;
  return o;
}
struct CamView {
  const float *R, *T, *focal, *pp;
  int row0, stripe_h, pitch;
  int h, W;
  int behind;
  float *origin_out;
  float *rays_out;
};
__host__ __device__ inline CamView no_camera() { return CamView{nullptr, nullptr, nullptr, nullptr, 0, 1, 0, 0, 0, 0, nullptr, nullptr}; }
struct CamK {
  Mat3 Ri;
  float ifx, ify, px, py;
};
__device__ __forceinline__ CamK cam_load(const CamView &c, const int b) {
  CamK k;
  k.Ri = inv3(c.R + 9 * b);
  k.ifx = 1.0f / c.focal[2 * b]; k.ify = 1.0f / c.focal[2 * b + 1];
  k.px = c.pp[2 * b]; k.py = c.pp[2 * b + 1];
  return k;
}
__device__ __forceinline__ int cam_irow(const CamView &c, const int i) {
  if (i < c.stripe_h) return c.row0 + i;
  int k = __float2int_rz(((float)i + 0.5f) * __builtin_amdgcn_rcpf((float)c.stripe_h));
  int r = i - k * c.stripe_h;
  if (r < 0) { --k; r += c.stripe_h; } else if (r >= c.stripe_h) { ++k; r -= c.stripe_h; }
  return c.row0 + k * c.pitch + r;
}
__device__ __forceinline__ void cam_ray(const CamK &k, const int ir, const int j, float &x, float &y, float &z) {
  const float vx = (k.px - ((float)j + 0.5f)) * k.ifx;
  const float vy = (k.py - ((float)ir + 0.5f)) * k.ify;
  const float wx = vx * k.Ri.m[0] + vy * k.Ri.m[3] + k.Ri.m[6];
  const float wy = vx * k.Ri.m[1] + vy * k.Ri.m[4] + k.Ri.m[7];
  const float wz = vx * k.Ri.m[2] + vy * k.Ri.m[5] + k.Ri.m[8];
  const float inv = __builtin_amdgcn_rsqf(wx * wx + wy * wy + wz * wz);
  x = wx * inv; y = wy * inv; z = wz * inv;
}
__device__ __forceinline__ void cam_origin(const CamK &k, const float *t, float &ox, float &oy, float &oz) {
  ox = -(t[0] * k.Ri.m[0] + t[1] * k.Ri.m[3] + t[2] * k.Ri.m[6]);
  oy = -(t[0] * k.Ri.m[1] + t[1] * k.Ri.m[4] + t[2] * k.Ri.m[7]);
  oz = -(t[0] * k.Ri.m[2] + t[1] * k.Ri.m[5] + t[2] * k.Ri.m[8]);
}

template <int NR>
__device__ __forceinline__ ConeRec block_cone256(const float (&rx)[NR], const float (&ry)[NR], const float (&rz)[NR],
                                                 const unsigned has, const int npx, float *red) {
  const int lane = threadIdx.x & 63, wave = threadIdx.x >> 6;
  float sx = 0.f, sy = 0.f, sz = 0.f, okf = 1.f;
#pragma unroll
  for (int k = 0; k < NR; ++k) {
    const float dn2 = fmaf(rz[k], rz[k], fmaf(ry[k], ry[k], rx[k] * rx[k]));
    const bool on = (has >> k) & 1u, fin = dn2 > 1e-30f && dn2 < 1e30f;
    sx += (on && fin) ? rx[k] : 0.f; sy += (on && fin) ? ry[k] : 0.f; sz += (on && fin) ? rz[k] : 0.f;
    okf = (on && !fin) ? 0.f : okf;
  }
  sx = wave_sum_dpp(sx); sy = wave_sum_dpp(sy); sz = wave_sum_dpp(sz); okf = wave_min(okf);
  if (lane == 0) { red[wave * 8 + 0] = sx; red[wave * 8 + 1] = sy; red[wave * 8 + 2] = sz; red[wave * 8 + 3] = okf; }
  __syncthreads();
  sx = red[0] + red[8] + red[16] + red[24];
  sy = red[1] + red[9] + red[17] + red[25];
  sz = red[2] + red[10] + red[18] + red[26];
  okf = fminf(fminf(red[3], red[11]), fminf(red[19], red[27]));
  const float n = sqrtf(fmaf(sz, sz, fmaf(sy, sy, sx * sx)));
  const float ax = sx / n, ay = sy / n, az = sz / n;
  float s2max = 0.f, cmin = 1.f;
#pragma unroll
  for (int k = 0; k < NR; ++k) {
    const float dn2 = fmaf(rz[k], rz[k], fmaf(ry[k], ry[k], rx[k] * rx[k]));
    const bool on = (has >> k) & 1u, fin = dn2 > 1e-30f && dn2 < 1e30f;
    const float inv = __builtin_amdgcn_rsqf(dn2);
    const float da = fmaf(rz[k], az, fmaf(ry[k], ay, rx[k] * ax));
    const float qx = fmaf(-da, ax, rx[k]), qy = fmaf(-da, ay, ry[k]), qz = fmaf(-da, az, rz[k]);
    const float s2 = fmaf(qz, qz, fmaf(qy, qy, qx * qx)) * (inv * inv);
    s2max = on ? fmaxf(s2max, fin ? s2 : 4.0f) : s2max;
    cmin = on ? fminf(cmin, fin ? da * inv : -1.0f) : cmin;
  }
  s2max = wave_max(s2max); cmin = wave_min(cmin);
  if (lane == 0) { red[wave * 8 + 4] = s2max; red[wave * 8 + 5] = cmin; }
  __syncthreads();
  s2max = fmaxf(fmaxf(red[4], red[12]), fmaxf(red[20], red[28]));
  cmin = fminf(fminf(red[5], red[13]), fminf(red[21], red[29]));
  const Cone c = cone_finish(ax, ay, az, n / (float)max(npx, 1), sqrtf(s2max) * (1.0f + 4e-7f) + 4e-7f, cmin - 4e-7f, okf != 0.f);
  return ConeRec{c.ax, c.ay, c.az, c.cs, c.sn, c.ok ? 1.f : 0.f, 0.f, 0.f};
}

struct ConeHierLds {
  float4 sum[16];
  float cnt[16];
  float ext[16][4];
};
constexpr int kConeRecsPerST = 21;
__host__ __device__ inline size_t cone_super_at(const size_t b, const size_t nst, const size_t st) { return b * nst * kConeRecsPerST + st; }
__host__ __device__ inline size_t cone_quad_at(const size_t b, const size_t nst, const size_t st, const int q) { return b * nst * kConeRecsPerST + nst + st * 4 + q; }
__host__ __device__ inline size_t cone_tile_at(const size_t b, const size_t nst, const size_t st, const int t) { return b * nst * kConeRecsPerST + nst * 5 + st * 16 + t; }
__host__ __device__ inline size_t cone_records(const size_t B, const size_t nst) { return B * nst * kConeRecsPerST; }
__device__ __forceinline__ void cone_thread_rays(const int t, int &lx0, int &ly) {
  const int lane = t & 63, j = lane & 15;
  lx0 = (lane >> 4) * 8 + (j & 1) * 4;
  ly = (t >> 6) * 8 + (j >> 1);
}
__device__ __forceinline__ float tile16_sum(float v) {
  v += VOGE_DPP(v, 0xB1); v += VOGE_DPP(v, 0x4E); v += VOGE_DPP(v, 0x141); v += VOGE_DPP(v, 0x140);
  return v;
}
__device__ __forceinline__ float tile16_max(float v) {
  v = fmaxf(v, VOGE_DPP(v, 0xB1)); v = fmaxf(v, VOGE_DPP(v, 0x4E)); v = fmaxf(v, VOGE_DPP(v, 0x141)); v = fmaxf(v, VOGE_DPP(v, 0x140));
  return v;
}
__device__ __forceinline__ float tile16_min(float v) {
  v = fminf(v, VOGE_DPP(v, 0xB1)); v = fminf(v, VOGE_DPP(v, 0x4E)); v = fminf(v, VOGE_DPP(v, 0x141)); v = fminf(v, VOGE_DPP(v, 0x140));
  return v;
}
__device__ __forceinline__ void block_cones_hier256(const float (&rx)[4], const float (&ry)[4], const float (&rz)[4], const unsigned has,
                                                    ConeRec *__restrict__ c_super, ConeRec *__restrict__ c_quad ,
                                                    ConeRec *__restrict__ c_tile , ConeHierLds &L) {
  const int t = threadIdx.x, lane = t & 63, wave = t >> 6;
  const int ltx = lane >> 4, tile = wave * 4 + ltx;
  float sx = 0.f, sy = 0.f, sz = 0.f, okf = 1.f, np = 0.f;
  float inv[4];
  bool fin[4];
#pragma unroll
  for (int k = 0; k < 4; ++k) {
    const float dn2 = fmaf(rz[k], rz[k], fmaf(ry[k], ry[k], rx[k] * rx[k]));
    const bool on = (has >> k) & 1u;
    fin[k] = dn2 > 1e-30f && dn2 < 1e30f;
    inv[k] = __builtin_amdgcn_rsqf(dn2);
    sx += (on && fin[k]) ? rx[k] : 0.f; sy += (on && fin[k]) ? ry[k] : 0.f; sz += (on && fin[k]) ? rz[k] : 0.f;
    okf = (on && !fin[k]) ? 0.f : okf;
    np += on ? 1.f : 0.f;
  }
  sx = tile16_sum(sx); sy = tile16_sum(sy); sz = tile16_sum(sz); okf = tile16_min(okf); np = tile16_sum(np);
  if ((lane & 15) == 0) { L.sum[tile] = make_float4(sx, sy, sz, okf); L.cnt[tile] = np; }
  __syncthreads();
  float ax[2], ay[2], az[2];
  {
    float gx = 0.f, gy = 0.f, gz = 0.f;
#pragma unroll
    for (int i = 0; i < 16; ++i) {
      const float4 v = L.sum[i];
      gx += v.x; gy += v.y; gz += v.z;
    }
    const float vx[2] = {sx, gx}, vy[2] = {sy, gy}, vz[2] = {sz, gz};
#pragma unroll
    for (int l = 0; l < 2; ++l) {
      const float rn = __builtin_amdgcn_rsqf(fmaf(vz[l], vz[l], fmaf(vy[l], vy[l], vx[l] * vx[l])));
      ax[l] = vx[l] * rn; ay[l] = vy[l] * rn; az[l] = vz[l] * rn;
    }
  }
  float s2m[2] = {0.f, 0.f}, cmn[2] = {1.f, 1.f};
#pragma unroll
  for (int k = 0; k < 4; ++k) {
    const bool on = (has >> k) & 1u;
#pragma unroll
    for (int l = 0; l < 2; ++l) {
      const float da = fmaf(rz[k], az[l], fmaf(ry[k], ay[l], rx[k] * ax[l]));
      const float qx = fmaf(-da, ax[l], rx[k]), qy = fmaf(-da, ay[l], ry[k]), qz = fmaf(-da, az[l], rz[k]);
      const float s2 = fmaf(qz, qz, fmaf(qy, qy, qx * qx)) * (inv[k] * inv[k]);
      s2m[l] = on ? fmaxf(s2m[l], fin[k] ? s2 : 4.0f) : s2m[l];
      cmn[l] = on ? fminf(cmn[l], fin[k] ? da * inv[k] : -1.0f) : cmn[l];
    }
  }
#pragma unroll
  for (int l = 0; l < 2; ++l) { s2m[l] = tile16_max(s2m[l]); cmn[l] = tile16_min(cmn[l]); }
// ... 338 lines not shown
```

Before: 4263 frames/s.

## Pack kernel arguments into structs and reload from kernarg to cut register pressure

Replaces the long parameter lists of the sweep and binB kernels with single argument structs read through the kernarg segment pointer. Values are re-fetched at late stages behind opaque asm barriers so the compiler does not keep them live in scalar or vector registers. It also adds occupancy hints to launch bounds, restructures the wide-path dispatch into a templated per-tile lambda, and rewrites the tie-break walk and the slice computation with cheaper selects and shifts. The aim is to lower register pressure and raise occupancy, at the cost of extra scalar loads and more fragile code.

```diff
diff --git a/voge_amd/csrc/sweep_iso.h b/voge_amd/csrc/sweep_iso.h
--- a/voge_amd/csrc/sweep_iso.h
+++ b/voge_amd/csrc/sweep_iso.h
@@ -39,16 +39,31 @@
 #endif
 constexpr int kExitGroup = VOGE_S2_EXIT_GROUP;
 
+struct SweepArgs {
+  const float4 *cull, *ms, *evr;
+  const float *rays;
+  const int *bin_count;
+  const int32_t *bin_id;
+  const float *bin_lb;
+  const int32_t *tl_id;
+  const float *tl_lb;
+  const int32_t *pool_id;
+  const float *pool_lb;
+  const int *tl_off;
+  const int2 *order;
+  int tiles_per_img, nstx, nst, N, H, W, K;
+  float thr_act;
+  int32_t *out_idx;
+  float *out_len, *out_act, *out_dsd;
+  int32_t *out_cnt;
+  CamView cam;
+};
 template <int GEN>
-__global__ void __launch_bounds__(64)
-sweep_iso_kernel(const float4 *__restrict__ cull, const float4 *__restrict__ ms, const float4 *__restrict__ evr, const float *__restrict__ rays,
-                 const int *__restrict__ bin_count, const int32_t *__restrict__ bin_id, const float *__restrict__ bin_lb,
-                 const int32_t *__restrict__ tl_id, const float *__restrict__ tl_lb, const int32_t *__restrict__ pool_id,
-                 const float *__restrict__ pool_lb, const int *__restrict__ tl_off, const int2 *__restrict__ order,
-                 const int tiles_per_img, const int nstx, const int nst, const int N, const int H, const int W, const int K,
-                 const float thr_act, int32_t *__restrict__ out_idx, float *__restrict__ out_len, float *__restrict__ out_act,
-                 float *__restrict__ out_dsd, int32_t *__restrict__ out_cnt,
-                 const CamView cam ) {
+__global__ void __launch_bounds__(64, GEN == 0 ? 3 : 2)
+sweep_iso_kernel(const SweepArgs ) {
+  const SweepArgs *A = arg_block<SweepArgs>();
+  const int K = A->K;
+  const float thr_act = A->thr_act;
   extern __shared__ __attribute__((aligned(16))) unsigned char smem_raw[];
   float *const Llen = reinterpret_cast<float *>(smem_raw);
   unsigned char *const Lpos_raw = smem_raw + sweep2_len_bytes(K);
@@ -58,7 +73,6 @@
   auto ghas = [](const int r) { return GEN != 2 || r < 2 || (r >= 5 && r < 8); };
 
   const int lane = threadIdx.x;
-  const int tiles_x = (W + 7) >> 3;
 #ifdef VOGE_SWEEP_TIMES
   const unsigned long long ts0 = wall_clock64();
   unsigned long long ts_fill = 0, ts_cons = 0, ts1 = 0, ts2 = 0;
@@ -66,89 +80,102 @@
   unsigned long long ts_slow = 0; unsigned st_slow = 0, st_lanes = 0, st_moved = 0, st_far = 0;
   int dbg_moved = 0;
 #endif
-  const int2 slot = order[blockIdx.x];
+  const int2 slot = A->order[blockIdx.x];
   if (slot.x < 0) return;
   if (slot.y == 0) {
-    if (out_act != nullptr) return;
+    if (A->out_act != nullptr) return;
     const int lin0 = slot.x & ~kPoolFlag;
-    const int b = lin0 / tiles_per_img, bx = lin0 - b * tiles_per_img;
+    const int b = lin0 / A->tiles_per_img, bx = lin0 - b * A->tiles_per_img, tiles_x = (A->W + 7) >> 3;
     const int ftx = bx % tiles_x, fty = bx / tiles_x;
-    const int tw = min(8, W - ftx * 8), th = min(8, H - fty * 8);
+    const int tw = min(8, A->W - ftx * 8), th = min(8, A->H - fty * 8);
     const int row_items = tw * K;
     if ((K & 3) == 0) {
       const int ipr = row_items >> 2;
       for (int it = lane; it < th * ipr; it += 64) {
         const int rr = it / ipr, j4 = it - rr * ipr;
-        const size_t o = (((size_t)b * H + fty * 8 + rr) * W + (size_t)ftx * 8) * K + (size_t)j4 * 4;
-        st16i<true>(out_idx + o, -1, -1, -1, -1);
-        st16f<true>(out_len + o, VOGE_SENT_LEN, VOGE_SENT_LEN, VOGE_SENT_LEN, VOGE_SENT_LEN);
+        const size_t o = (((size_t)b * A->H + fty * 8 + rr) * A->W + (size_t)ftx * 8) * K + (size_t)j4 * 4;
+        st16i<true>(A->out_idx + o, -1, -1, -1, -1);
+        st16f<true>(A->out_len + o, VOGE_SENT_LEN, VOGE_SENT_LEN, VOGE_SENT_LEN, VOGE_SENT_LEN);
       }
     } else {
       for (int it = lane; it < th * row_items; it += 64) {
         const int rr = it / row_items, j = it - rr * row_items;
-        const size_t o = (((size_t)b * H + fty * 8 + rr) * W + (size_t)ftx * 8) * K + j;
-        out_idx[o] = -1; out_len[o] = VOGE_SENT_LEN;
+        const size_t o = (((size_t)b * A->H + fty * 8 + rr) * A->W + (size_t)ftx * 8) * K + j;
+        A->out_idx[o] = -1; A->out_len[o] = VOGE_SENT_LEN;
       }
     }
-    if (out_cnt != nullptr) {
+    if (A->out_cnt != nullptr) {
       const int rr = lane >> 3, x = lane & 7;
-      if (rr < th && x < tw) out_cnt[((size_t)b * H + fty * 8 + rr) * W + (size_t)ftx * 8 + x] = 0;
+      if (rr < th && x < tw) A->out_cnt[((size_t)b * A->H + fty * 8 + rr) * A->W + (size_t)ftx * 8 + x] = 0;
     }
-    if (cam.R != nullptr && cam.rays_out != nullptr) {
+    if (A->cam.R != nullptr && A->cam.rays_out != nullptr) {
       const int rr = lane >> 3, x = lane & 7;
       if (rr < th && x < tw) {
-        const CamK ck = cam_load(cam, b);
+        const CamK ck = cam_load(A->cam, b);
         float ex, ey, ez;
-        cam_ray(ck, cam_irow(cam, fty * 8 + rr), ftx * 8 + x, ex, ey, ez);
-        float *o = cam.rays_out + (((size_t)b * H + fty * 8 + rr) * W + (size_t)ftx * 8 + x) * 3;
+        cam_ray(ck, cam_irow(A->cam, fty * 8 + rr), ftx * 8 + x, ex, ey, ez);
+        float *o = A->cam.rays_out + (((size_t)b * A->H + fty * 8 + rr) * A->W + (size_t)ftx * 8 + x) * 3;
         o[0] = ex; o[1] = ey; o[2] = ez;
       }
     }
     return;
   }
+  bool wide = false;
+  if (A->N > 65536) {
+    const int lin = slot.x & ~kPoolFlag;
+    const int b = lin / A->tiles_per_img, bx = lin - b * A->tiles_per_img, tiles_x = (A->W + 7) >> 3;
+    const int tx = bx % tiles_x, ty = bx / tiles_x;
+    const int bin = (b * A->nst + ((ty * 8) / kST) * A->nstx + (tx * 8) / kST) * 4 + (((ty * 8) / kQuad) & 1) * 2 + (((tx * 8) / kQuad) & 1);
+    const int bc = (slot.y >= 0) ? slot.y : ((A->bin_count != nullptr) ? A->bin_count[bin] : -1);
+    wide = bc < 0 || bc > 65536;
+  }
+  auto tile = [&](auto wide_tag, const int pass, int slot_x, int slot_y, int K) {
+  asm volatile("" : "+s"(slot_x), "+s"(slot_y), "+s"(K));
+  A = arg_block<SweepArgs>(true);
+  const int2 slot = make_int2(slot_x, slot_y);
   const bool pooled = (slot.x & kPoolFlag) != 0;
   const int lin = slot.x & ~kPoolFlag;
-  const int b = lin / tiles_per_img, bx = lin - b * tiles_per_img;
+  const int b = lin / A->tiles_per_img, bx = lin - b * A->tiles_per_img, tiles_x = (A->W + 7) >> 3;
   const int tx = bx % tiles_x, ty = bx / tiles_x;
-  const int bin = (b * nst + ((ty * 8) / kST) * nstx + (tx * 8) / kST) * 4 + (((ty * 8) / kQuad) & 1) * 2 + (((tx * 8) / kQuad) & 1);
+  const int bin = (b * A->nst + ((ty * 8) / kST) * A->nstx + (tx * 8) / kST) * 4 + (((ty * 8) / kQuad) & 1) * 2 + (((tx * 8) / kQuad) & 1);
   const int tc = slot.y;
-  const int bc = (tc >= 0) ? tc : ((bin_count != nullptr) ? bin_count[bin] : -1);
+  const int bc = (tc >= 0) ? tc : ((A->bin_count != nullptr) ? A->bin_count[bin] : -1);
   const bool binned = bc >= 0;
-  const int src_n = binned ? bc : N;
-  const size_t list_at = pooled ? (size_t)tl_off[lin] : (size_t)lin * kTileCap;
-  const int32_t *src_id = (tc >= 0) ? (pooled ? pool_id : tl_id) + list_at : (binned ? bin_id + (size_t)bin * kQCap : nullptr);
-  const float *src_lb = (tc >= 0) ? (pooled ? pool_lb : tl_lb) + list_at : (binned ? bin_lb + (size_t)bin * kQCap : nullptr);
+  const int src_n = binned ? bc : A->N;
+  const size_t list_at = pooled ? (size_t)A->tl_off[lin] : (size_t)lin * kTileCap;
+  const int32_t *src_id = (tc >= 0) ? (pooled ? A->pool_id : A->tl_id) + list_at : (binned ? A->bin_id + (size_t)bin * kQCap : nullptr);
+  const float *src_lb = (tc >= 0) ? (pooled ? A->pool_lb : A->tl_lb) + list_at : (binned ? A->bin_lb + (size_t)bin * kQCap : nullptr);
   const bool pref = tc >= 0;
-  const float4 *cullb = cull + (size_t)b * N;
-  const float4 *msb = ms + (size_t)b * N;
+  const float4 *cullb = A->cull + (size_t)b * A->N;
+  const float4 *msb = A->ms + (size_t)b * A->N;
   const float4 rec_none = make_float4(0.f, 0.f, 0.f, INFINITY);
   const float4 cull_none = make_float4(0.f, 0.f, 0.f, -1.f);
-  const bool h_is_id = (N <= 65536) || !binned;
+  const bool h_is_id = (A->N <= 65536) || !binned;
   auto id_of = [&](const unsigned h) -> int { return h_is_id ? (int)h : src_id[h]; };
   const float not_full = __uint_as_float(__float_as_uint(VOGE_SENT_LEN) - 1u);
   if (lane < kS2Pad) { S.x[64 + lane] = 0.f; S.y[64 + lane] = 0.f; S.z[64 + lane] = 0.f; S.a[64 + lane] = INFINITY; }
   if (GEN && lane < kS2Pad) G.e[0][64 + lane] = __uint_as_float(0x7fc00000u);
-  const float4 *evrb = GEN ? evr + (size_t)b * N * 3 : nullptr;
+  const float4 *evrb = GEN ? A->evr + (size_t)b * A->N * 3 : nullptr;
   bool tile_gen = false;
 
   Cone wcone;
   bool unit_rays = false;
   wcone.ok = false;
-  const bool from_cam = cam.R != nullptr;
+  const bool from_cam = A->cam.R != nullptr;
   CamK ck;
-  if (from_cam) ck = cam_load(cam, b);
+  if (from_cam) ck = cam_load(A->cam, b);
   auto ray_of = [&](const int x, const int y, float &rx, float &ry, float &rz) {
     if (from_cam) {
-      cam_ray(ck, cam_irow(cam, y), x, rx, ry, rz);
+      cam_ray(ck, cam_irow(A->cam, y), x, rx, ry, rz);
     } else {
-      const size_t rid = ((size_t)b * H + y) * W + x;
-      rx = rays[3 * rid + 0]; ry = rays[3 * rid + 1]; rz = rays[3 * rid + 2];
+      const size_t rid = ((size_t)b * A->H + y) * A->W + x;
+      rx = A->rays[3 * rid + 0]; ry = A->rays[3 * rid + 1]; rz = A->rays[3 * rid + 2];
     }
   };
   auto ray_setup = [&](const bool mine, const float mdx, const float mdy, const float mdz) {
     const int px = tx * 8 + (lane & 7), py = ty * 8 + (lane >> 3);
     float ox_ = mdx, oy_ = mdy, oz_ = mdz;
-    if (!mine) ray_of(min(px, W - 1), min(py, H - 1), ox_, oy_, oz_);
+    if (!mine) ray_of(min(px, A->W - 1), min(py, A->H - 1), ox_, oy_, oz_);
     const RayDir u = ray_dir(ox_, oy_, oz_);
     unit_rays = __all(!u.ok || u.unit);
     wcone.ok = false;
@@ -168,20 +195,20 @@
     const int r = WIDE ? pass * 32 + (lane & 31) : lane;
     const int col = WIDE ? (lane & 31) : lane;
     const int px = tx * 8 + (r & 7), py = ty * 8 + (r >> 3);
-    const bool valid = (px < W) && (py < H) && (!WIDE || lane < 32);
-    const size_t ray_id = ((size_t)b * H + min(py, H - 1)) * W + min(px, W - 1);
+    const bool valid = (px < A->W) && (py < A->H) && (!WIDE || lane < 32);
+    const size_t ray_id = ((size_t)b * A->H + min(py, A->H - 1)) * A->W + min(px, A->W - 1);
     int id0 = (lane < src_n) ? (binned ? src_id[lane] : lane) : -1;
     float lb0 = (binned && lane < src_n) ? src_lb[lane] : -INFINITY;
     int id1 = (64 + lane < src_n) ? (binned ? src_id[64 + lane] : 64 + lane) : -1;
     float lb1 = (binned && 64 + lane < src_n) ? src_lb[64 + lane] : -INFINITY;
     float dx, dy, dz;
-    ray_of(min(px, W - 1), min(py, H - 1), dx, dy, dz);
-    if (from_cam && cam.rays_out != nullptr && valid) {
-      float *o = cam.rays_out + 3 * ray_id;
+    ray_of(min(px, A->W - 1), min(py, A->H - 1), dx, dy, dz);
+    if (from_cam && A->cam.rays_out != nullptr && valid) {
+      float *o = A->cam.rays_out + 3 * ray_id;
       o[0] = dx; o[1] = dy; o[2] = dz;
     }
-    const __amdgpu_buffer_rsrc_t rs_ms = out_rsrc(const_cast<float4 *>(msb), (unsigned)N * 16u),
-                                 rs_cull = out_rsrc(const_cast<float4 *>(cullb), (unsigned)N * 16u);
+    const __amdgpu_buffer_rsrc_t rs_ms = out_rsrc(const_cast<float4 *>(msb), (unsigned)A->N * 16u),
+                                 rs_cull = out_rsrc(const_cast<float4 *>(cullb), (unsigned)A->N * 16u);
     auto load_ms = [&](const int id) {
       const voge_v4f r = __builtin_amdgcn_raw_buffer_load_b128(rs_ms, id * 16, 0, 0);
       return make_float4(r[0], r[1], r[2], (id >= 0) ? r[3] : INFINITY);
@@ -190,7 +217,7 @@
       const voge_v4f r = __builtin_amdgcn_raw_buffer_load_b128(rs_cull, id * 16, 0, 0);
       return make_float4(r[0], r[1], r[2], (id >= 0) ? r[3] : -1.f);
     };
-    const __amdgpu_buffer_rsrc_t rs_ev = out_rsrc(const_cast<float4 *>(GEN ? evrb : msb), GEN ? (unsigned)N * 48u : 0u);
+    const __amdgpu_buffer_rsrc_t rs_ev = out_rsrc(const_cast<float4 *>(GEN ? evrb : msb), GEN ? (unsigned)A->N * 48u : 0u);
     auto load_ev = [&](const int id, const int k) {
       const voge_v4f r = __builtin_amdgcn_raw_buffer_load_b128(rs_ev, id * 48 + 16 * k, 0, 0);
       return make_float4(r[0], r[1], r[2], r[3]);
@@ -199,7 +226,7 @@
     float4 c0 = pref ? cull_none : load_cull(id0);
     float4 ea0 = rec_none, ea1 = rec_none, ea2 = rec_none;
     if (GEN) { ea0 = load_ev(id0, 0); ea1 = load_ev(id0, 1); ea2 = load_ev(id0, 2); }
-    if (pass == 0) ray_setup(!WIDE, dx, dy, dz);
+    ray_setup(!WIDE, dx, dy, dz);
     const float rdn2 = __builtin_amdgcn_rcpf((dx * dx + dy * dy) + dz * dz);
     float *const mylen = Llen + col;
     uint16_t *const mypos16 = reinterpret_cast<uint16_t *>(Lpos_raw) + col;
@@ -285,18 +312,20 @@
       const int pos0 = pos;
       float top = len;
       bool walking = go, first = true;
+      const int go_v = fresh_v(go ? 1 : 0), full_v = fresh_v(full ? 1 : 0);
       while (__ballot(walking) != 0ull) {
         const int r1 = max(pos - 1, 0), r2 = max(pos - 2, 0), r3 = max(pos - 3, 0), r4 = max(pos - 4, 0);
         const float l1 = len_at(r1), l2 = len_at(r2), l3 = len_at(r3), l4 = len_at(r4);
         const unsigned h1 = pos_at(r1), h2 = pos_at(r2), h3 = pos_at(r3), h4 = pos_at(r4);
-        bool g1 = l1 > len, g2 = l2 > len, g3 = l3 > len, g4 = l4 > len;
+        float k1 = l1, k2 = l2, k3 = l3, k4 = l4;
         if (__builtin_expect(__ballot(walking & ((l1 == len) | (l2 == len) | (l3 == len) | (l4 == len))) != 0ull, 0)) {
           if (walking & ((l1 == len) | (l2 == len) | (l3 == len) | (l4 == len))) {
             if (my_id < 0) my_id = id_of(p);
-            g1 = g1 | ((l1 == len) && id_of(h1) > my_id); g2 = g2 | ((l2 == len) && id_of(h2) > my_id);
-            g3 = g3 | ((l3 == len) && id_of(h3) > my_id); g4 = g4 | ((l4 == len) && id_of(h4) > my_id);
+            k1 = ((l1 == len) && id_of(h1) > my_id) ? INFINITY : k1; k2 = ((l2 == len) && id_of(h2) > my_id) ? INFINITY : k2;
+            k3 = ((l3 == len) && id_of(h3) > my_id) ? INFINITY : k3; k4 = ((l4 == len) && id_of(h4) > my_id) ? INFINITY : k4;
           }
         }
+        const bool g1 = k1 > len, g2 = k2 > len, g3 = k3 > len, g4 = k4 > len;
         const bool c1 = walking & (pos >= 1) & g1, c2 = c1 & (pos >= 2) & g2, c3 = c2 & (pos >= 3) & g3, c4 = c3 & (pos >= 4) & g4;
         if (first) top = c1 ? l1 : len;
         first = false;
@@ -307,9 +336,9 @@
         pos -= (c1 ? 1 : 0) + (c2 ? 1 : 0) + (c3 ? 1 : 0) + (c4 ? 1 : 0);
         walking = c4;
       }
-      put(go ? pos : Kv, len, p);
-      if (go) {
-        if (full) {
+      put(go_v != 0 ? pos : Kv, len, p);
+      if (go_v != 0) {
+        if (full_v != 0) {
           tailf = top; worstf = top;
         } else {
           if (pos == pos0) tailf = len;
@@ -556,6 +585,12 @@
     ts2 = wall_clock64();
 #endif
 
+    A = arg_block<SweepArgs>(true);
+    const int H = A->H, W = A->W, N = A->N;
+    int32_t *const out_idx = A->out_idx, *const out_cnt = A->out_cnt;
+    float *const out_len = A->out_len, *const out_act = A->out_act, *const out_dsd = A->out_dsd;
+    const float *const rays = A->rays;
+    const float4 *const ms = A->ms, *const evr = A->evr;
     __syncthreads();
     S.cnt[lane] = valid ? cnt : 0;
     if (out_cnt != nullptr && valid) out_cnt[((size_t)b * H + py) * W + px] = cnt;
@@ -702,7 +737,7 @@
         }
       }
     } else {
-      constexpr int kOddU = 8;
+      constexpr int kOddU = WIDE ? 4 : 8;
       const float inv_ri = 1.0f / (float)max(row_items, 1), invK = 1.0f / (float)K;
       const int nit = th * row_items;
       const size_t tile_pix = ((size_t)b * H + ty * 8 + row0) * W + (size_t)tx * 8;
@@ -772,13 +807,16 @@
     }
   };
 
-  if ((h_is_id ? N : src_n) <= 65536) {
-    run(std::false_type{}, 0);
+  run(wide_tag, pass);
+  };
+  if (!wide) {
+    tile(std::false_type{}, 0, slot.x, slot.y, K);
   } else {
-    run(std::true_type{}, 0);
-    run(std::true_type{}, 1);
+    tile(std::true_type{}, 0, slot.x, slot.y, K);
+    tile(std::true_type{}, 1, slot.x, slot.y, K);
   }
 #ifdef VOGE_SWEEP_TIMES
+  const int b = (slot.x & ~kPoolFlag) / A->tiles_per_img, bx = (slot.x & ~kPoolFlag) - b * A->tiles_per_img;
   if (lane == 0 && b == 0 && bx < 8192) {
     unsigned long long *o = g_sweep_times + 8 * (size_t)bx;
     o[0] = ts0; o[1] = ts1; o[2] = ts_fill; o[3] = ts_cons; o[4] = ts2; o[5] = wall_clock64(); o[6] = ((unsigned long long)blockIdx.x << 32) | st_eval;
diff --git a/voge_amd/csrc/trace_bin.h b/voge_amd/csrc/trace_bin.h
--- a/voge_amd/csrc/trace_bin.h
+++ b/voge_amd/csrc/trace_bin.h
@@ -128,7 +128,8 @@
 
 __host__ __device__ inline bool deal_interleaved(const int N) { return N < kParts * kBinThreads; }
 __device__ __forceinline__ int slice_of(const int g, const int N) {
-  return deal_interleaved(N) ? g % kParts : (g / kBinThreads) % kParts;
+  static_assert((kParts & (kParts - 1)) == 0 && kBinThreads == 1024, "powers of two");
+  return (int)(((unsigned)g >> (deal_interleaved(N) ? 0 : 10)) & (unsigned)(kParts - 1));
 }
 
 template <bool ISO_PREP>
@@ -421,6 +422,7 @@
   unsigned ovf;
   int count;
   int nflag;
+  int wg[2];
   int spill;
   float tc[kTilesPerQuad][8];
   int toff[kTilesPerQuad];
@@ -480,7 +482,7 @@
     }
     bin_test_batch<ELL>(S, gid, c, sink);
   }
-  if (S.n_ext > 0) {
+  if (fresh_s(S.n_ext) > 0) {
     const int *extn = segn + (kParts + 1), *exto = S.exto;
     for (int base = 0; base < S.n_ext; base += kQT * kGU) {
       int gid[kGU];
@@ -587,32 +589,60 @@
   return Kk.flagged ? fminf(lb_sphere, ord2f(bmin[qb])) : lb_sphere;
 }
 
+struct BinBArgs {
+  const float4 *cull, *ell;
+  const int *seg_count;
+  const int32_t *seg_id;
+  const float4 *seg_rec;
+  const ConeRec *cones;
+  int N, H, W, nstx, nsty, nbin_total;
+  int *q_count;
+  int32_t *q_id;
+  float *q_lb;
+  int *tl_count;
+  int32_t *tl_id;
+  float *tl_lb;
+  int2 *order;
+  unsigned long long *pool_top;
+  int pool_cap;
+  int32_t *pool_id;
+  float *pool_lb;
+  int *tl_off;
+  const int *seg_ext;
+  const int32_t *ext_id;
+  int K;
+  int32_t *out_idx;
+  float *out_len, *out_act, *out_dsd;
+  int32_t *out_cnt;
+  float *out_weight;
+  int64_t *out_valid;
+  CamView cam;
+};
+
 struct BinLong {
   BinStream S;
   BinKeys Kk;
   Cone tcone;
   bool tile_ok;
   int tile, quad, total;
-  unsigned long long *pool_top;
-  int *tl_off, *tl_count, *q_count;
-  const int *seg_ext;
   int bin;
-  int pool_cap;
-  int32_t *pool_id;
-  float *pool_lb;
   int2 *my_order;
 };
 template <bool ELL>
 __device__ __forceinline__ void binB_long_path(const BinLong A, BinLds &L) {
-  const int tid = threadIdx.x, lane = tid & 63, wave = tid >> 6;
-  const BinStream &S = A.S;
+  int tid = threadIdx.x;
+  asm volatile("" : "+v"(tid));
+  const int lane = tid & 63, wave = tid >> 6;
+  BinStream S = A.S;
+  S.n_src = fresh_v(S.n_src); S.ovf = (unsigned)fresh_v((int)S.ovf); S.n_ext = fresh_s(S.n_ext); S.N = fresh_s(S.N);
+  const BinBArgs *P = arg_block<BinBArgs>(true);
   const int total = A.total;
   __syncthreads();
   for (int i = tid; i < kTilesPerQuad * kBuckets; i += kQT) (&L.hist4[0][0])[i] = 0;
-  if (S.n_ext > 0) {
+  if (fresh_s(S.n_ext) > 0) {
     const int p = tid / kExtChunks, q = tid % kExtChunks;
     const int ne = L.extn[p + 1] - L.extn[p];
-    L.exto[p][q] = (q * kExtChunk < ne) ? A.seg_ext[((size_t)A.bin * kParts + p) * kExtChunks + q] : 0;
+    L.exto[p][q] = (q * kExtChunk < ne) ? P->seg_ext[((size_t)A.bin * kParts + p) * kExtChunks + q] : 0;
   }
   if (lane == 0) {
     L.tc[wave][0] = A.tcone.ax; L.tc[wave][1] = A.tcone.ay; L.tc[wave][2] = A.tcone.az; L.tc[wave][3] = A.tcone.cs;
@@ -620,8 +650,8 @@
     L.tc[wave][6] = A.tile_ok ? 1.0f : 0.0f;
   }
   if (tid == 0) {
-    const unsigned long long at64 = atomicAdd(A.pool_top, (unsigned long long)total);
-    int at = (at64 + (unsigned long long)total <= (unsigned long long)A.pool_cap) ? (int)at64 : -1;
+    const unsigned long long at64 = atomicAdd(P->pool_top, (unsigned long long)total);
+    int at = (at64 + (unsigned long long)total <= (unsigned long long)P->pool_cap) ? (int)at64 : -1;
     L.toff[0] = at;
     L.count = 0;
   }
@@ -630,8 +660,8 @@
   bool pooled = surv_at >= 0;
   int tile_n[kTilesPerQuad] = {0, 0, 0, 0};
   if (pooled) {
-    int32_t *sv_id = A.pool_id + surv_at;
-    float *sv_key = A.pool_lb + surv_at;
+    int32_t *sv_id = P->pool_id + surv_at;
+    float *sv_key = P->pool_lb + surv_at;
     bin_stream_sources<ELL>(S, L.segn, tid, [&](const int (&g)[kGU], const float4 (&cj)[kGU], const bool (&kp)[kGU],
                                             const bool (&el)[kGU], const float (&gkey)[kGU]) {
       int slot[kGU];
@@ -647,6 +677,7 @@
     __threadfence_block();
     __syncthreads();
     BIN_TS(1, 2);
+    P = arg_block<BinBArgs>(true);
     auto tile_mask = [&](const size_t g, const float4 cj, const bool el) {
       unsigned mk = 0u;
 #pragma unroll 1
@@ -692,8 +723,8 @@
     if (ELL && A.Kk.flagged) bin_bmin_suffix(L.bmin, L.wsum, tid);
     if (tid == 0) {
       const int need = tile_n[0] + tile_n[1] + tile_n[2] + tile_n[3];
-      const unsigned long long at64 = (need > 0) ? atomicAdd(A.pool_top, (unsigned long long)need) : 0ull;
-      int at = (at64 + (unsigned long long)need <= (unsigned long long)A.pool_cap) ? (int)at64 : -1;
+      const unsigned long long at64 = (need > 0) ? atomicAdd(P->pool_top, (unsigned long long)need) : 0ull;
+      int at = (at64 + (unsigned long long)need <= (unsigned long long)P->pool_cap) ? (int)at64 : -1;
 #pragma unroll
       for (int t = 0; t < kTilesPerQuad; ++t) { L.toff[t] = at; if (at >= 0) at += tile_n[t]; }
     }
@@ -701,6 +732,8 @@
     pooled = L.toff[0] >= 0;
     BIN_TS(1, 3);
     if (pooled) {
+      int32_t *const pool_id = P->pool_id;
+      float *const pool_lb = P->pool_lb;
       for (int i = tid; i < total; i += kQT) {
         const uint32_t word = (uint32_t)sv_id[i];
         const size_t g = word & 0x7fffffffu;
@@ -714,16 +747,17 @@
         for (int t = 0; t < kTilesPerQuad; ++t) {
           if ((mk >> t) & 1u) {
             const size_t pos = (size_t)L.toff[t] + (size_t)atomicAdd(&L.hist4[t][q], 1);
-            A.pool_id[pos] = (int32_t)g;
-            A.pool_lb[pos] = lbv;
+            pool_id[pos] = (int32_t)g;
+            pool_lb[pos] = lbv;
           }
         }
       }
     }
   }
+  P = arg_block<BinBArgs>(true);
   if (lane == 0 && A.tile_ok) {
-    A.tl_count[A.tile] = pooled ? tile_n[wave] : -1;
-    A.tl_off[A.tile] = pooled ? L.toff[wave] : -1;
+    P->tl_count[A.tile] = pooled ? tile_n[wave] : -1;
+    P->tl_off[A.tile] = pooled ? L.toff[wave] : -1;
   }
   __syncthreads();
   if (lane == 0) L.wsum[wave] = A.tile_ok ? (pooled ? tile_n[wave] : 0x7fffffff) : -1;
@@ -737,7 +771,7 @@
     }
     A.my_order[slot] = make_int2(A.tile_ok ? (pooled ? (A.tile | kPoolFlag) : A.tile) : -1, pooled ? mine : -1);
   }
-  if (tid == 0) A.q_count[A.quad] = pooled ? -2 : -1;
+  if (tid == 0) P->q_count[A.quad] = pooled ? -2 : -1;
   BIN_TS(1, 4);
 }
 
@@ -747,47 +781,37 @@
 #endif
 template <bool ELL>
 __global__ void __launch_bounds__(kQT) __attribute__((amdgpu_waves_per_eu(VOGE_BINB_WPE, VOGE_BINB_WPE)))
-binB_kernel(const float4 *__restrict__ cull, const float4 *__restrict__ ell, const int *__restrict__ seg_count,
-            const int32_t *__restrict__ seg_id, const float4 *__restrict__ seg_rec,
-            const ConeRec *__restrict__ cones ,
-            const int N, const int H, const int W,
-            const int nstx, const int nsty, const int nbin_total,
-            int *__restrict__ q_count, int32_t *__restrict__ q_id, float *__restrict__ q_lb,
-            int *__restrict__ tl_count, int32_t *__restrict__ tl_id, float *__restrict__ tl_lb,
-            int2 *__restrict__ order ,
-            unsigned long long *__restrict__ pool_top, const int pool_cap, int32_t *__restrict__ pool_id, float *__restrict__ pool_lb,
-            int *__restrict__ tl_off, const int *__restrict__ seg_ext, const int32_t *__restrict__ ext_id,
-            const int K, int32_t *__restrict__ out_idx, float *__restrict__ out_len, float *__restrict__ out_act,
-            float *__restrict__ out_dsd, int32_t *__restrict__ out_cnt, float *__restrict__ out_weight,
-            int64_t *__restrict__ out_valid, const CamView cam ) {
+binB_kernel(const BinBArgs ) {
   __shared__ BinLds L;
-  const int tid = threadIdx.x, lane = tid & 63, wave = tid >> 6;
+  const BinBArgs *P = arg_block<BinBArgs>();
+  int tid = threadIdx.x, lane = tid & 63, wave = tid >> 6;
+#define BINB_RETID() do { asm volatile("" : "+v"(tid)); lane = tid & 63; wave = tid >> 6; } while (0)
   BIN_TS(1, 7);
   const int b = blockIdx.y;
   const int binl = blockIdx.x >> 2, qq = blockIdx.x & 3;
-  const int stx = binl % nstx, sty = binl / nstx;
-  const int bin = b * nstx * nsty + binl;
+  const int stx = binl % P->nstx, sty = binl / P->nstx;
+  const int bin = b * P->nstx * P->nsty + binl;
   const int quad = bin * 4 + qq;
-  const int tiles_x = (W + 7) >> 3, tiles_y = (H + 7) >> 3;
+  const int tiles_x = (P->W + 7) >> 3, tiles_y = (P->H + 7) >> 3;
   const int tx = stx * (kST / 8) + (qq & 1) * 2 + (wave & 1), ty = sty * (kST / 8) + (qq >> 1) * 2 + (wave >> 1);
   const bool tile_ok = tx < tiles_x && ty < tiles_y;
   const int tile = b * tiles_x * tiles_y + ty * tiles_x + tx;
 
   ConeRec tcr, qcr;
-  if (cam.R != nullptr) {
-    const CamK ck = cam_load(cam, b);
-    cam_two_cones(ck, cam, tx * 8, ty * 8, 8, stx * kST + (qq & 1) * kQuad, sty * kST + (qq >> 1) * kQuad, kQuad, tcr, qcr);
+  if (P->cam.R != nullptr) {
+    const CamK ck = cam_load(P->cam, b);
+    cam_two_cones(ck, P->cam, tx * 8, ty * 8, 8, stx * kST + (qq & 1) * kQuad, sty * kST + (qq >> 1) * kQuad, kQuad, tcr, qcr);
   } else {
-    tcr = cones[cone_tile_at(b, (size_t)nstx * nsty, binl, ((qq >> 1) * 2 + (wave >> 1)) * 4 + (qq & 1) * 2 + (wave & 1))];
-    qcr = cones[cone_quad_at(b, (size_t)nstx * nsty, binl, qq)];
-  }
-  const int my_cnt = (tid < kParts) ? seg_count[(size_t)bin * kParts + tid] : 0;
-  const bool ranked = nbin_total <= kRankMaxBins;
-  const int4 est0 = (ranked && tid < nbin_total) ? *reinterpret_cast<const int4 *>(seg_count + (size_t)tid * kParts) : make_int4(0, 0, 0, 0);
-  const int4 est_mine = ranked ? *reinterpret_cast<const int4 *>(seg_count + (size_t)bin * kParts) : make_int4(0, 0, 0, 0);
+    tcr = P->cones[cone_tile_at(b, (size_t)P->nstx * P->nsty, binl, ((qq >> 1) * 2 + (wave >> 1)) * 4 + (qq & 1) * 2 + (wave & 1))];
+    qcr = P->cones[cone_quad_at(b, (size_t)P->nstx * P->nsty, binl, qq)];
+  }
+  const int my_cnt = (tid < kParts) ? P->seg_count[(size_t)bin * kParts + tid] : 0;
+  const bool ranked = P->nbin_total <= kRankMaxBins;
+  const int4 est0 = (ranked && tid < P->nbin_total) ? *reinterpret_cast<const int4 *>(P->seg_count + (size_t)tid * kParts) : make_int4(0, 0, 0, 0);
+  const int4 est_mine = ranked ? *reinterpret_cast<const int4 *>(P->seg_count + (size_t)bin * kParts) : make_int4(0, 0, 0, 0);
   const Cone tcone = load_cone(tcr), qcone = load_cone(qcr);
   {
-    if (tid == 0) { L.count = 0; L.nflag = 0; L.spill = 0; }
+    if (tid == 0) { L.count = 0; L.nflag = 0; L.spill = 0; L.wg[0] = blockIdx.x; L.wg[1] = blockIdx.y; }
     if (wave == 0) {
       int c = (lane < kParts) ? my_cnt : 0;
       const unsigned long long ofm = __ballot(lane < kParts && c < 0);
@@ -809,11 +833,12 @@
       static_assert(kParts * kExtChunks == kQT, "one thread per (slice, chunk)");
       const int p = tid / kExtChunks, q = tid % kExtChunks;
       const int ne = L.extn[p + 1] - L.extn[p];
-      L.exto[p][q] = (q * kExtChunk < ne) ? seg_ext[((size_t)bin * kParts + p) * kExtChunks + q] : 0;
+      L.exto[p][q] = (q * kExtChunk < ne) ? P->seg_ext[((size_t)bin * kParts + p) * kExtChunks + q] : 0;
     };
-    if (L.extn[kParts] > 0) load_ext_tables();
+    if (__builtin_amdgcn_readfirstlane(L.extn[kParts]) > 0) load_ext_tables();
   }
   BIN_TS(1, 0);
+  BINB_RETID();
 
   BIN_TS(1, 6);
   int rank = bin;
@@ -821,11 +846,12 @@
     auto est_of = [](const int4 v) {
       return (v.x < 0 ? kSegCap : v.x) + (v.y < 0 ? kSegCap : v.y) + (v.z < 0 ? kSegCap : v.z) + (v.w < 0 ? kSegCap : v.w);
     };
+    const int *const seg_count = P->seg_count;
     auto estimate = [&](const int q) { return est_of(*reinterpret_cast<const int4 *>(seg_count + (size_t)q * kParts)); };
     if (ranked) {
       const int mine = est_of(est_mine);
       int ahead = 0;
-      for (int q = tid; q < nbin_total; q += kQT) {
+      for (int q = tid; q < P->nbin_total; q += kQT) {
         const int e = (q == tid) ? est_of(est0) : estimate(q);
         ahead += (e > mine || (e == mine && q < bin)) ? 1 : 0;
       }
@@ -836,19 +862,19 @@
       __syncthreads();
     }
   }
-  int2 *my_order = order + (size_t)rank * kTilesPerBin + qq * kTilesPerQuad;
+  int2 *my_order = P->order + (size_t)rank * kTilesPerBin + qq * kTilesPerQuad;
   const int n_src = L.segn[kParts];
   const unsigned ovf = L.ovf;
-  const float4 *cullb = cull + (size_t)b * N;
-  const float4 *ellb = ell + (size_t)b * N * 2;
-  const int32_t *segs = seg_id + (size_t)bin * kParts * kSegCap;
-  const float4 *segr = seg_rec + (size_t)bin * kParts * kSegCap;
+  const float4 *cullb = P->cull + (size_t)b * P->N;
+  const float4 *ellb = P->ell + (size_t)b * P->N * 2;
+  const int32_t *segs = P->seg_id + (size_t)bin * kParts * kSegCap;
+  const float4 *segr = P->seg_rec + (size_t)bin * kParts * kSegCap;
   float rmax = 0.0f;
   float klo = INFINITY, khi = -INFINITY;
   bool any_el = false;
   BinStream S;
-  S.cullb = cullb; S.ellb = ellb; S.segr = segr; S.segs = segs; S.n_src = n_src; S.N = N; S.ovf = ovf; S.qcone = qcone;
-  S.ext_id = ext_id; S.n_ext = L.extn[kParts]; S.exto = &L.exto[0][0];
+  S.cullb = cullb; S.ellb = ellb; S.segr = segr; S.segs = segs; S.n_src = n_src; S.N = P->N; S.ovf = ovf; S.qcone = qcone;
+  S.ext_id = P->ext_id; S.n_ext = __builtin_amdgcn_readfirstlane(L.extn[kParts]); S.exto = &L.exto[0][0];
   bin_stream_sources<ELL>(S, L.segn, tid, [&](const int (&g)[kGU], const float4 (&cj)[kGU], const bool (&kp)[kGU],
                                           const bool (&el)[kGU], const float (&gkey)[kGU]) {
     int slot[kGU];
@@ -865,10 +891,11 @@
     }
   });
   BIN_TS(1, 1);
+  BINB_RETID();
   if (__any(any_el) && lane == 0) L.nflag = 1;
   float hi = wave_max(khi), lo = wave_min(klo), rm = wave_max(rmax);
   if (lane == 0) { L.red[wave * 8 + 0] = hi; L.red[wave * 8 + 1] = lo; L.red[wave * 8 + 2] = rm; }
-  if (S.n_ext > 0) __syncthreads();
+  if (fresh_s(S.n_ext) > 0) __syncthreads();
   for (int i = tid; i < kBuckets; i += kQT) { L.hist[i] = 0; L.bmin[i] = f2ord(INFINITY); }
   __syncthreads();
   const int total = L.count;
@@ -884,8 +911,7 @@
   if (__builtin_expect(total > kQCap, 0)) {
     BinLong A;
     A.S = S; A.Kk = Kk; A.tcone = tcone; A.tile_ok = tile_ok; A.tile = tile; A.quad = quad; A.total = total;
-    A.pool_top = pool_top; A.tl_off = tl_off; A.tl_count = tl_count; A.q_count = q_count; A.pool_cap = pool_cap;
-    A.pool_id = pool_id; A.pool_lb = pool_lb; A.my_order = my_order; A.seg_ext = seg_ext; A.bin = bin;
+    A.my_order = my_order; A.bin = bin;
     binB_long_path<ELL>(A, L);
   } else {
   for (int i = tid; i < total; i += kQT) {
@@ -913,6 +939,7 @@
   }
   __syncthreads();
   BIN_TS(1, 2);
+  BINB_RETID();
   for (int i = tid; i < total; i += kQT) {
     const uint64_t kk = L.keys[i];
     L.sorted[atomicAdd(&L.hist[bucket_of(kk)], 1)] = (uint32_t)kk;
@@ -937,6 +964,7 @@
   }
   __syncthreads();
   BIN_TS(1, 3);
+  BINB_RETID();
   auto len_bound = [&](const uint32_t word, const float4 cr) {
     const float v = (ELL && (word & 0x80000000u)) ? fmaf(cr.z, qcone.az, fmaf(cr.y, qcone.ay, cr.x * qcone.ax)) + 0.0f
                                          : depth_key(cr, qcone);
@@ -945,8 +973,8 @@
 
   int kept = 0;
   if (tile_ok) {
-    int32_t *oid = tl_id + (size_t)tile * kTileCap;
-    float *olb = tl_lb + (size_t)tile * kTileCap;
+    int32_t *oid = P->tl_id + (size_t)tile * kTileCap;
+    float *olb = P->tl_lb + (size_t)tile * kTileCap;
     BIN_WTS(0);
 #ifndef VOGE_BINB_FU
 #define VOGE_BINB_FU 4
@@ -989,13 +1017,14 @@
     }
     BIN_WTS(1);
     if (lane == 0) {
-      if (kept > kTileCap) { tl_count[tile] = -1; L.spill = 1; }
-      else tl_count[tile] = kept;
+      if (kept > kTileCap) { P->tl_count[tile] = -1; L.spill = 1; }
+      else P->tl_count[tile] = kept;
     }
   }
   if (lane == 0) L.wsum[wave] = tile_ok ? min(kept, kTileCap + 1) : -1;
   __syncthreads();
   BIN_TS(1, 4);
+  BINB_RETID();
   if (lane == 0) {
     const int mine = L.wsum[wave];
     int slot = 0;
@@ -1006,8 +1035,8 @@
     my_order[slot] = make_int2(tile_ok ? tile : -1, (mine > kTileCap) ? -1 : mine);
   }
   if (L.spill) {
-    int32_t *oid = q_id + (size_t)quad * kQCap;
-    float *olb = q_lb + (size_t)quad * kQCap;
+    int32_t *oid = P->q_id + (size_t)quad * kQCap;
+    float *olb = P->q_lb + (size_t)quad * kQCap;
     for (int i = tid; i < total; i += kQT) {
       const uint32_t word = L.sorted[i];
       oid[i] = (int32_t)(word & 0x7fffffffu);
@@ -1016,9 +1045,20 @@
       olb[i] = len_bound(word, crec);
     }
   }
-  if (tid == 0) q_count[quad] = L.spill ? total : -2;
-  }
-  for (int w = 0; w < kTilesPerQuad && out_idx != nullptr; ++w) {
+  if (tid == 0) P->q_count[quad] = L.spill ? total : -2;
+  }
+  P = arg_block<BinBArgs>(true);
+  int32_t *const out_idx = P->out_idx;
+  if (out_idx != nullptr) {
+  const int H = P->H, W = P->W, K = P->K;
+  const int bix = __builtin_amdgcn_readfirstlane(L.wg[0]), b = __builtin_amdgcn_readfirstlane(L.wg[1]);
+  int tid = threadIdx.x;
+  asm volatile("" : "+v"(tid));
+  const int qq = bix & 3, stx = (bix >> 2) % P->nstx, sty = (bix >> 2) / P->nstx;
+  float *const out_len = P->out_len, *const out_act = P->out_act, *const out_dsd = P->out_dsd, *const out_weight = P->out_weight;
+  int32_t *const out_cnt = P->out_cnt;
+  int64_t *const out_valid = P->out_valid;
+  for (int w = 0; w < kTilesPerQuad; ++w) {
     if (L.wsum[w] != 0) continue;
     const int ftx = stx * (kST / 8) + (qq & 1) * 2 + (w & 1), fty = sty * (kST / 8) + (qq >> 1) * 2 + (w >> 1);
     const int tw = min(8, W - ftx * 8), th = min(8, H - fty * 8);
@@ -1053,7 +1093,9 @@
       if (x < tw && out_valid != nullptr) out_valid[pix] = 0;
     }
   }
+  }
   BIN_TS(1, 5);
-}
-
-}
+#undef BINB_RETID
+}
+
+}
diff --git a/voge_amd/csrc/trace_fwd.hip b/voge_amd/csrc/trace_fwd.hip
--- a/voge_amd/csrc/trace_fwd.hip
+++ b/voge_amd/csrc/trace_fwd.hip
@@ -1106,11 +1106,11 @@
     if (rc) return rc;
   }
 #endif
-  hipLaunchKernelGGL(binB_kernel<!ISO>, dim3(ws.nstx * ws.nsty * 4, B), dim3(kQT), 0, st, ws.cull, ws.ell, ws.seg_count, ws.seg_id, ws.seg_rec,
-                     cones, N, H, W, ws.nstx, ws.nsty, ws.nbin, ws.q_count, ws.q_id, ws.q_lb, ws.tl_count, ws.tl_id, ws.tl_lb,
-                     ws.order, ws.pool_top, ws.pool_cap, ws.pool_id, ws.pool_lb, ws.tl_off, ws.seg_ext, ws.ext_id, K,
-                     (v2 && act == nullptr) ? nullptr : idx , len, act, dsd, cnt,
-                     nullptr, nullptr, cam);
+  const BinBArgs ba{ws.cull, ws.ell, ws.seg_count, ws.seg_id, ws.seg_rec, cones, N, H, W, ws.nstx, ws.nsty, ws.nbin, ws.q_count, ws.q_id, ws.q_lb,
+                    ws.tl_count, ws.tl_id, ws.tl_lb, ws.order, ws.pool_top, ws.pool_cap, ws.pool_id, ws.pool_lb, ws.tl_off, ws.seg_ext, ws.ext_id, K,
+                    (v2 && act == nullptr) ? nullptr : idx , len, act, dsd, cnt,
+                    nullptr, nullptr, cam};
+  hipLaunchKernelGGL(binB_kernel<!ISO>, dim3(ws.nstx * ws.nsty * 4, B), dim3(kQT), 0, st, ba);
   {
     int rc = launch_status();
     if (rc) return rc;
@@ -1118,9 +1118,9 @@
   const int2 *order = ws.order;
   dim3 grid(ws.nbin * kTilesPerBin);
   if (v2) {
-    hipLaunchKernelGGL(sweep, grid, dim3(T), lds2, st, ws.cull, ws.ms, ws.evr, rays, ws.q_count, ws.q_id, ws.q_lb, ws.tl_id,
-                       ws.tl_lb, ws.pool_id, ws.pool_lb, ws.tl_off, order, ((W + 7) / 8) * ((H + 7) / 8), ws.nstx, ws.nstx * ws.nsty, N, H, W, K,
-                       thr_act, idx, len, act, dsd, cnt, cam);
+    const SweepArgs sa{ws.cull, ws.ms, ws.evr, rays, ws.q_count, ws.q_id, ws.q_lb, ws.tl_id, ws.tl_lb, ws.pool_id, ws.pool_lb, ws.tl_off,
+                       order, ((W + 7) / 8) * ((H + 7) / 8), ws.nstx, ws.nstx * ws.nsty, N, H, W, K, thr_act, idx, len, act, dsd, cnt, cam};
+    hipLaunchKernelGGL(sweep, grid, dim3(T), lds2, st, sa);
     return launch_status();
   }
 #ifdef VOGE_AB
diff --git a/voge_amd/csrc/voge_common.h b/voge_amd/csrc/voge_common.h
--- a/voge_amd/csrc/voge_common.h
+++ b/voge_amd/csrc/voge_common.h
@@ -432,6 +432,21 @@
   float *rays_out;
 };
 __host__ __device__ inline CamView no_camera() { return CamView{nullptr, nullptr, nullptr, nullptr, 0, 1, 0, 0, 0, 0, nullptr, nullptr}; }
+template <class T>
+__device__ __forceinline__ const T *arg_block(const bool again = false) {
+  typedef const T __attribute__((address_space(4))) *CP;
+  unsigned long long v = (unsigned long long)__builtin_amdgcn_kernarg_segment_ptr();
+  if (again) asm volatile("" : "+s"(v));
+  return (const T *)(CP)v;
+}
+__device__ __forceinline__ int fresh_s(int v) {
+  asm volatile("" : "+s"(v));
+  return v;
+}
+__device__ __forceinline__ int fresh_v(int v) {
+  asm volatile("" : "+v"(v));
+  return v;
+}
 struct CamK {
   Mat3 Ri;
   float ifx, ify, px, py;
```

Result: no change. 4284 frames/s (median of 6 runs) (+0.5%).
